# bg5sbk/dragonboat

Measured on AMD Instinct MI355X. Metric: quorum-commit decisions/sec (whole node) + % HBM roofline at 1/2/4/8 GPUs, higher is better.
Workload: dtype u64

## Files before the change

dragonboat_amd/csrc/hq_dstep_k.h:

```cpp
#pragma once

#include <chrono>
#include <cstdlib>

#include "hq_dstep.h"
#include "hq_internal.h"

namespace hq {
struct StepArgs {};
struct JobArgs {};
}

namespace {

enum List { kCommits, kReady, kResps, kStates, kDropped, kDeferred, kFallback, kDecisions,
            kRerun, kEvents, kSlotted, kLists };
enum InputError : uint32_t { kErrHandle = 1, kErrOffsets = 2, kErrBoffsets = 4, kErrTwice = 8,
                             kErrScan = 16, kErrTicket = 32 };
constexpr uint32_t kTickets = 8;

struct StepK : hq::StepArgs {
    hq_dgroup *groups;
    hq_dmember *members;
    hq_dread *reads;
    uint64_t n;
    uint64_t i_begin, i_end;
    uint64_t n_handles;
    uint64_t n_events, n_bytes;
    uint32_t *stamp;
    uint32_t step_no;
    uint32_t *error;
    uint32_t *wide;
    const uint32_t *handles;
    const uint64_t *offsets;
    const hq_event *events;
    const uint64_t *boffsets;
    const uint8_t *bytes;
    const uint64_t *prefix;
    uint64_t own_lo, own_hi;
    uint32_t *counts;
    uint32_t *wsum;
    uint64_t ws;
    const uint32_t *scan;
    uint64_t nw;
    uint32_t *pre;
    char *out;
    const struct Layout *layout;
    hq_dgroup *groups_old;
    uint64_t *match_old;
    hq_dread *reads_old;
    uint32_t spec_col, spec_valid;
    uint8_t *rerun;
    hq_ready_to_read *ready_slot;
    uint32_t *rerun_list;
    uint64_t out_cap;
    uint32_t allow_column, pad_j;
    struct Layout *host_layout;
    const uint32_t *sizes;
    const uint32_t *sizes_src;
    uint64_t *bsum;
    uint32_t spec_ready, chunk;
    uint64_t ready_off;
    uint32_t *ready_wide;
    uint64_t *tiles;
    uint32_t *tickets;
    const uint16_t *sizes16;
    const uint16_t *sizes16_src;
    uint32_t bytes_only;
    uint32_t slots;
    uint64_t slot_off, cnt_off;
    uint32_t test_scan_fail, pad_t;
};

constexpr uint32_t kSlotTile = 256;
constexpr uint64_t kSlotTileBytes = kSlotTile * sizeof(hq_ready_compact);
static_assert(kSlotTileBytes % 256 == 0, "slot tiles keep the region's 256-byte alignment");

struct Layout {
    uint64_t off[kLists];
    uint32_t len[kLists];
    uint64_t total;
    uint32_t error, overflow;
    uint32_t commit_column;
    uint32_t ready_compact;
    uint32_t pad;
    uint64_t reserve;
};
constexpr uint32_t kColumn64 = 1, kColumn32 = 2;
constexpr uint32_t kReadyCompact = 4;
constexpr uint32_t kReadySlots = 8;

constexpr uint32_t kTileVal = (1u << 28) - 1;

constexpr uint32_t kMaxJobs = kDStepMaxJobs;
struct JobMap : hq::JobArgs {
    const StepK *ks;
    uint32_t job0, count;
    uint32_t blk0[kMaxJobs + 1];
    uint32_t *tickets;
    uint32_t chunk;
    StepK *table_out;
    uint32_t bsum_scanned, pad;
};
static_assert(sizeof(StepK) % 8 == 0, "k_size_sums copies the table in 8-byte words");

__device__ __forceinline__ uint32_t job_of(const JobMap &m, uint32_t b) {
    uint32_t j = 0;
    while (j + 1 < m.count && b >= m.blk0[j + 1]) ++j;
    return j;
}

constexpr int kMaxChunks = 4;
constexpr int kMaxJobChunks = 8;
static_assert(kMaxChunks <= kMaxJobChunks, "the chunk events serve both paths");
static_assert(kMaxJobChunks <= kTickets, "a ticket word per pass A launch");
constexpr uint64_t kChunkGroups = 65536;
__host__ __device__ inline uint64_t slot_layout(uint64_t n, uint64_t *slot_off, uint64_t *cnt_off) {
    const uint64_t tiles = (n + kSlotTile - 1) / kSlotTile;
    const uint64_t so = (n * 4 + 255) & ~uint64_t(255);
    const uint64_t co = so + tiles * kSlotTileBytes;
    if (slot_off) *slot_off = so;
    if (cnt_off) *cnt_off = co;
    return co + ((tiles * 4 + 255) & ~uint64_t(255));
}

constexpr int kScanT = 1024, kScanE = 11;
constexpr uint64_t kScanSmall = 2 * kScanT * kScanE;

constexpr uint32_t kSizeTile = 1024;
constexpr uint64_t kSizeApplyDirect = 2048;

template <class K, class... A>
int launch(hq_ctx *ctx, hipStream_t s, const char *what, K k, uint64_t grid, unsigned block,
           const A &...a) {
    hipLaunchKernelGGL(k, dim3((unsigned)grid), dim3(block), 0, s, a...);
    return hq::check_hip(ctx, hipGetLastError(), what);
}

}

namespace hq {
int launch_step(hq_ctx *ctx, bool write, bool stream, bool small, const StepArgs &k);
int launch_step_jobs(hq_ctx *ctx, bool write, bool small, const JobArgs &m);
int launch_step_lite(hq_ctx *ctx, hipStream_t s, const StepArgs &k);
int launch_step_lite_jobs(hq_ctx *ctx, hipStream_t s, const JobArgs &m);
int launch_step_restore(hq_ctx *ctx, hipStream_t s, const StepArgs &k);
int launch_layout(hq_ctx *ctx, hipStream_t s, const StepArgs &k);
int launch_scan_layout(hq_ctx *ctx, hipStream_t s, const StepArgs &k);
int launch_scan_layout_jobs(hq_ctx *ctx, hipStream_t s, const JobArgs &m);
int launch_size_sums(hq_ctx *ctx, hipStream_t s, const JobArgs &m);
int launch_bsum_scan_jobs(hq_ctx *ctx, hipStream_t s, const JobArgs &m);
int launch_size_apply(hq_ctx *ctx, hipStream_t s, const JobArgs &m);
int scan_wave_sums(hq_ctx *ctx, hipStream_t s, void *tmp, size_t *tmp_bytes, uint32_t *wsum,
                   uint32_t *scan, size_t ws);
int scan_sizes(hq_ctx *ctx, hipStream_t s, void *tmp, size_t *tmp_bytes, const void *sizes,
               bool s16, uint64_t n, uint64_t *prefix);
inline uint64_t now_ns() {
    using namespace std::chrono;
    return (uint64_t)duration_cast<nanoseconds>(steady_clock::now().time_since_epoch()).count();
}
inline bool env_flag(const char *name) {
    const char *v = std::getenv(name);
    return v && std::atoi(v) != 0;
}
int grow(hq_ctx *ctx, void **p, size_t *cap, size_t need, bool keep, const char *what);
template <class T>
int grow(hq_ctx *ctx, T **p, size_t *cap, size_t need, bool keep, const char *what) {
    return grow(ctx, reinterpret_cast<void **>(p), cap, need, keep, what);
}
int stamp_clock(hq_dstep *d, hipStream_t s, int slot);
int wait_stream(hq_dstep *d, hipStream_t s, const char *what);
}

struct hq_dstep {
    hq_ctx *ctx = nullptr;
    bool test_fail_regrow = false;
    bool test_scan_fail = false;
    hq_dgroup *groups = nullptr;
    hq_dread *reads = nullptr;
    hq_dmember *members = nullptr;
    hq_dgroup *groups_old = nullptr;
    hq_dread *reads_old = nullptr;
    uint64_t *match_old = nullptr;
    uint8_t *rerun = nullptr;
    uint32_t *rerun_list = nullptr;
    hq_ready_to_read *ready_slot = nullptr;
    size_t rcap = 0;
    uint32_t *stamp = nullptr;
    uint64_t gcap = 0, mcap = 0;
    uint64_t n_groups = 0;
    uint32_t max_members = 0;
    uint32_t step_no = 0;
    uint32_t commit_column = 0;
    void *in = nullptr;
    size_t in_cap = 0;
    uint32_t *counts = nullptr, *scan = nullptr, *bases = nullptr;
    size_t cnt_cap = 0;
    uint32_t *wsum = nullptr;
    size_t wsum_cap = 0;
    bool wsum_dirty = true;
    void *scan_tmp = nullptr;
    size_t scan_tmp_cap = 0;
    void *host_out = nullptr;
    size_t host_out_cap = 0;
    Layout *layout = nullptr;
    Layout *host_layout = nullptr;
    hipStream_t copy = nullptr;
    hipEvent_t ev_in[kMaxJobChunks] = {};
    hipStream_t copy2 = nullptr;
    hipEvent_t ev_in2[kMaxJobChunks] = {};
    char *bounce = nullptr;
    hipEvent_t bounce_ev[2] = {nullptr, nullptr};
    hipEvent_t ev_sync = nullptr;
    hipEvent_t ev_t0 = nullptr, ev_t1 = nullptr;
    StepK *jobs_host = nullptr, *jobs_dev = nullptr;
    const StepK *jobs_host_dev = nullptr;
    uint32_t jobs_cap = 0;
    uint32_t *tickets = nullptr;
    bool tickets_dirty = false;
    uint64_t *tiles = nullptr;
    size_t tiles_cap = 0;
    uint32_t wait_mode = HQ_WAIT_BLOCK, wait_poll_us = 50, wait_sleep_us = 20;
    uint64_t wait_pred_ns = 0;
    bool wait_clock = false;
    uint64_t *clock_host = nullptr;
    hq_wait_clock last_wait{};
};
```

dragonboat_amd/csrc/hq_dstep_layout.hip:

```cpp
#include <hipcub/hipcub.hpp>

#include "hq_dstep_k.h"

namespace {

struct PackSize {
    const uint32_t *sizes;
    uint64_t n;
    const uint16_t *sizes16 = nullptr;
    __host__ __device__ uint64_t operator()(uint64_t i) const {
        if (sizes16) return i < n ? sizes16[i] : 0;
        const uint32_t s = i < n ? sizes[i] : 0;
        return (uint64_t)(s & 0xFFFFu) << 32 | (s >> 16);
    }
};

__device__ void layout_from(const uint32_t *bnd, uint64_t n, uint32_t *error, uint64_t cap,
                            uint32_t allow_column, uint64_t want_events, Layout *lay,
                            Layout *host_lay) {
    uint32_t *wide = error + 1;
    uint32_t *ready_wide = error + 2;
    if (want_events != ~uint64_t(0) && (uint64_t)(bnd[kEvents + 1] - bnd[kEvents]) != want_events)
        *error |= kErrBoffsets;
    lay->ready_compact = (allow_column & kReadyCompact) && !*ready_wide;
    const uint64_t rec[kLists] = {sizeof(hq_commit_event),
                                  lay->ready_compact ? sizeof(hq_ready_compact) : sizeof(hq_ready_to_read),
                                  sizeof(hq_read_index_resp), sizeof(hq_state_change),
                                  sizeof(hq_dropped_read), 8, 8, 0, 0, 0, 0};
    const uint32_t commits = bnd[1] - bnd[0];
    lay->commit_column = (allow_column & kColumn32) && !*wide && 4 * (uint64_t)commits > n
                             ? kColumn32
                         : (allow_column & kColumn64) && 2 * (uint64_t)commits > n ? kColumn64 : 0;
    const bool slots = (allow_column & kReadySlots) != 0;
    const uint64_t reserve = slots ? slot_layout(n, nullptr, nullptr) : 0;
    uint64_t total = reserve;
    for (int l = 0; l < kLists; ++l) {
        const uint32_t len = bnd[l + 1] - bnd[l];
        lay->len[l] = len;
        if (l == kCommits && slots && lay->commit_column == kColumn32) {
            lay->off[l] = 0;
            continue;
        }
        lay->off[l] = total;
        const uint64_t bytes = l == kCommits && lay->commit_column
                                   ? n * (lay->commit_column == kColumn32 ? 4 : 8)
                                   : len * rec[l];
        total += (bytes + 255) & ~uint64_t(255);
    }
    lay->total = total;
    lay->reserve = reserve;
    lay->error = *error;
    lay->overflow = total > cap;
    if (!((lay->overflow && !*error) || *error == kErrScan)) {
        *error = 0;
        *wide = 0;
        *ready_wide = 0;
    }
    *host_lay = *lay;
}

__global__ void k_layout(const uint32_t *scan, uint64_t n, uint64_t nw, uint32_t *error,
                         uint64_t cap, uint32_t allow_column, uint64_t want_events, Layout *lay,
                         Layout *host_lay) {
    if (threadIdx.x != 0) return;
    uint32_t bnd[kLists + 1];
    for (int l = 0; l <= kLists; ++l) bnd[l] = scan[(uint64_t)l * nw];
    layout_from(bnd, n, error, cap, allow_column, want_events, lay, host_lay);
}

__device__ __forceinline__ void scan_layout(const uint32_t *wsum, uint32_t *scan, uint64_t ws,
                                            uint64_t n, uint64_t nw, uint32_t *error, uint64_t cap,
                                            uint32_t allow_column, uint64_t want_events, Layout *lay,
                                            Layout *host_lay) {
    __shared__ uint32_t tile[kScanT * kScanE];
    __shared__ uint32_t wtot[kScanT / 64];
    __shared__ uint32_t bnd[kLists + 1];
    const int t = threadIdx.x, lane = t & 63, wv = t >> 6;
    uint32_t carry = 0;
    for (uint64_t base = 0; base < ws; base += (uint64_t)kScanT * kScanE) {
        for (int k = 0; k < kScanE; ++k) {
            const uint64_t j = base + (uint64_t)k * kScanT + t;
            tile[k * kScanT + t] = j < ws ? wsum[j] : 0u;
        }
        __syncthreads();
        uint32_t v[kScanE], sum = 0;
        for (int k = 0; k < kScanE; ++k) {
            v[k] = tile[t * kScanE + k];
            sum += v[k];
        }
        uint32_t x = sum;
        for (int d = 1; d < 64; d <<= 1) {
            const uint32_t y = __shfl_up(x, d, 64);
            x += lane >= d ? y : 0u;
        }
        if (lane == 63) wtot[wv] = x;
        __syncthreads();
        uint32_t before = 0, all = 0;
        for (int w = 0; w < kScanT / 64; ++w) {
            const uint32_t z = wtot[w];
            before += w < wv ? z : 0u;
            all += z;
        }
        uint32_t run = carry + before + x - sum;
        for (int k = 0; k < kScanE; ++k) {
            tile[t * kScanE + k] = run;
            run += v[k];
        }
        __syncthreads();
        for (int k = 0; k < kScanE; ++k) {
            const uint64_t j = base + (uint64_t)k * kScanT + t;
            if (j < ws) {
                const uint32_t e = tile[k * kScanT + t];
                scan[j] = e;
                if (j % nw == 0 && j / nw <= kLists) bnd[j / nw] = e;
            }
        }
        carry += all;
        __syncthreads();
    }
    if (t == 0) layout_from(bnd, n, error, cap, allow_column, want_events, lay, host_lay);
}

__global__ __launch_bounds__(kScanT) void k_scan_layout(const uint32_t *wsum, uint32_t *scan,
                                                        uint64_t ws, uint64_t n, uint64_t nw,
                                                        uint32_t *error, uint64_t cap,
                                                        uint32_t allow_column, uint64_t want_events,
                                                        Layout *lay, Layout *host_lay) {
    scan_layout(wsum, scan, ws, n, nw, error, cap, allow_column, want_events, lay, host_lay);
}

__host__ __device__ inline uint64_t want_events_of(const StepK &a) {
    return a.bytes_only ? a.n_events : ~uint64_t(0);
}

__global__ __launch_bounds__(kScanT) void k_scan_layout_jobs(const StepK *ks) {
    const StepK &a = ks[blockIdx.x];
    scan_layout(a.wsum, const_cast<uint32_t *>(a.scan), a.ws, a.n, a.nw, a.error, a.out_cap,
                a.allow_column, want_events_of(a), const_cast<Layout *>(a.layout), a.host_layout);
}

__device__ __forceinline__ uint64_t packed_size(const StepK &a, uint64_t i) {
    if (i >= a.n) return 0;
    if (a.bytes_only) return a.sizes16[i];
    const uint32_t s = a.sizes[i];
    return (uint64_t)(s & 0xFFFFu) << 32 | (s >> 16);
}

__device__ __forceinline__ uint64_t block_excl_scan(uint64_t v, uint64_t *total) {
    __shared__ uint64_t wt[1024 / 64];
    const int lane = threadIdx.x & 63, wv = threadIdx.x >> 6;
    uint64_t x = v;
#pragma unroll
    for (int d = 1; d < 64; d <<= 1) {
        const uint64_t y = __shfl_up(x, d, 64);
        x += lane >= d ? y : 0ull;
    }
    if (lane == 63) wt[wv] = x;
    __syncthreads();
    uint64_t before = 0, all = 0;
    for (int w = 0; w < (int)(blockDim.x / 64); ++w) {
        before += w < wv ? wt[w] : 0ull;
        all += wt[w];
    }
    __syncthreads();
    *total = all;
    return before + x - v;
}

__global__ __launch_bounds__(256) void k_size_sums(const JobMap m) {
    if (m.table_out && blockIdx.x == 0) {
        const uint64_t *src = reinterpret_cast<const uint64_t *>(m.ks + m.job0);
        uint64_t *dst = reinterpret_cast<uint64_t *>(m.table_out + m.job0);
        for (uint32_t q = threadIdx.x; q < m.count * (uint32_t)(sizeof(StepK) / 8); q += 256)
            dst[q] = src[q];
    }
    const uint32_t j = job_of(m, blockIdx.x);
    const StepK &a = m.ks[m.job0 + j];
    const uint64_t b = blockIdx.x - m.blk0[j], i0 = b * kSizeTile + threadIdx.x * 4;
    uint64_t v = 0;
    if (a.bytes_only && a.sizes16_src) {
        uint16_t *dst = const_cast<uint16_t *>(a.sizes16);
        uint16_t z[4];
        if (i0 + 4 <= a.n && !(reinterpret_cast<uintptr_t>(a.sizes16_src) & 7)) {
            const uint64_t w = *reinterpret_cast<const uint64_t *>(a.sizes16_src + i0);
#pragma unroll
            for (int k = 0; k < 4; ++k) z[k] = (uint16_t)(w >> (16 * k));
            *reinterpret_cast<uint64_t *>(dst + i0) = w;
        } else {
#pragma unroll
            for (int k = 0; k < 4; ++k) {
                const uint64_t i = i0 + k;
                z[k] = i < a.n ? a.sizes16_src[i] : 0;
                if (i < a.n) dst[i] = z[k];
            }
        }
#pragma unroll
        for (int k = 0; k < 4; ++k) v += z[k];
    } else if (!a.bytes_only && a.sizes_src) {
        uint32_t *dst = const_cast<uint32_t *>(a.sizes);
#pragma unroll
        for (int k = 0; k < 4; ++k) {
            const uint64_t i = i0 + k;
            const uint32_t z = i < a.n ? a.sizes_src[i] : 0;
            if (i < a.n) dst[i] = z;
            v += (uint64_t)(z & 0xFFFFu) << 32 | (z >> 16);
        }
    } else {
#pragma unroll
        for (int k = 0; k < 4; ++k) v += packed_size(a, i0 + k);
    }
    uint64_t tot;
    (void)block_excl_scan(v, &tot);
    if (threadIdx.x == 0) a.bsum[b] = tot;
}

__global__ __launch_bounds__(1024) void k_bsum_scan_jobs(const JobMap m) {
    const StepK &a = m.ks[m.job0 + blockIdx.x];
    const uint64_t nb = (a.n + 1 + kSizeTile - 1) / kSizeTile;
    uint64_t carry = 0;
    for (uint64_t base = 0; base < nb; base += 1024) {
        const uint64_t k = base + threadIdx.x;
        const uint64_t v = k < nb ? a.bsum[k] : 0;
        uint64_t tot;
        const uint64_t ex = block_excl_scan(v, &tot);
        if (k < nb) a.bsum[k] = carry + ex;
        carry += tot;
    }
}

__global__ __launch_bounds__(256) void k_size_apply(const JobMap m) {
    const uint32_t j = job_of(m, blockIdx.x);
    const StepK &a = m.ks[m.job0 + j];
    const uint64_t b = blockIdx.x - m.blk0[j], i0 = b * kSizeTile + threadIdx.x * 4;
    uint64_t base;
    if (m.bsum_scanned) {
        base = a.bsum[b];
    } else {
        uint64_t before = 0;
        for (uint64_t k = threadIdx.x; k < b; k += 256) before += a.bsum[k];
        (void)block_excl_scan(before, &base);
    }
    uint64_t v[4], sum = 0;
#pragma unroll
    for (int k = 0; k < 4; ++k) {
        v[k] = packed_size(a, i0 + k);
        sum += v[k];
    }
    uint64_t tot;
    uint64_t run = base + block_excl_scan(sum, &tot);
    uint64_t *prefix = const_cast<uint64_t *>(a.prefix);
#pragma unroll
    for (int k = 0; k < 4; ++k) {
        if (i0 + k <= a.n) prefix[i0 + k] = run;
        run += v[k];
    }
}

}

namespace hq {

int launch_layout(hq_ctx *ctx, hipStream_t s, const StepArgs &ka) {
    const StepK &k = static_cast<const StepK &>(ka);
    return launch(ctx, s, "k_layout", k_layout, 1, 64, k.scan, k.n, k.nw, k.error, k.out_cap,
                  k.allow_column, want_events_of(k), const_cast<Layout *>(k.layout), k.host_layout);
}
int launch_scan_layout(hq_ctx *ctx, hipStream_t s, const StepArgs &ka) {
    const StepK &k = static_cast<const StepK &>(ka);
    return launch(ctx, s, "k_scan_layout", k_scan_layout, 1, kScanT, k.wsum,
                  const_cast<uint32_t *>(k.scan), k.ws, k.n, k.nw, k.error, k.out_cap,
                  k.allow_column, want_events_of(k), const_cast<Layout *>(k.layout), k.host_layout);
}
int launch_scan_layout_jobs(hq_ctx *ctx, hipStream_t s, const JobArgs &ma) {
    const JobMap &m = static_cast<const JobMap &>(ma);
    return launch(ctx, s, "k_scan_layout_jobs", k_scan_layout_jobs, m.count, kScanT, m.ks);
}
int launch_size_sums(hq_ctx *ctx, hipStream_t s, const JobArgs &ma) {
    const JobMap &m = static_cast<const JobMap &>(ma);
    return launch(ctx, s, "k_size_sums", k_size_sums, m.blk0[m.count], 256, m);
}
int launch_bsum_scan_jobs(hq_ctx *ctx, hipStream_t s, const JobArgs &ma) {
    const JobMap &m = static_cast<const JobMap &>(ma);
    return launch(ctx, s, "k_bsum_scan_jobs", k_bsum_scan_jobs, m.count, 1024, m);
}
int launch_size_apply(hq_ctx *ctx, hipStream_t s, const JobArgs &ma) {
    const JobMap &m = static_cast<const JobMap &>(ma);
    return launch(ctx, s, "k_size_apply", k_size_apply, m.blk0[m.count], 256, m);
}

int scan_wave_sums(hq_ctx *ctx, hipStream_t s, void *tmp, size_t *tmp_bytes, uint32_t *wsum,
                   uint32_t *scan, size_t ws) {
    return check_hip(ctx, hipcub::DeviceScan::ExclusiveSum(tmp, *tmp_bytes, wsum, scan, ws, s),
                     tmp ? "hipcub scan" : "hipcub scan size");
}
int scan_sizes(hq_ctx *ctx, hipStream_t s, void *tmp, size_t *tmp_bytes, const void *sizes,
               bool s16, uint64_t n, uint64_t *prefix) {
    const hipcub::TransformInputIterator<uint64_t, PackSize, hipcub::CountingInputIterator<uint64_t>>
        packed_sizes(hipcub::CountingInputIterator<uint64_t>(0),
                     PackSize{static_cast<const uint32_t *>(sizes), n,
                              s16 ? static_cast<const uint16_t *>(sizes) : nullptr});
    return check_hip(ctx, hipcub::DeviceScan::ExclusiveSum(tmp, *tmp_bytes, packed_sizes, prefix,
                                                           n + 1, s),
                     tmp ? "hipcub scan" : "hipcub scan size");
}

}
```

dragonboat_amd/csrc/hq_dstep_step.hip:

```cpp
#include "hq_dstep_k.h"
#include "hq_launch.h"

namespace {

__device__ __forceinline__ bool is_response(uint32_t t) {
    return t == HQ_MSG_REPLICATE_RESP || t == HQ_MSG_REQUEST_VOTE_RESP ||
           t == HQ_MSG_HEARTBEAT_RESP || t == 20 || t == 8 || t == 9;
}

struct ByteReader {
    const uint8_t *p, *end;
    uintptr_t wa = 1;
    uint64_t w = 0;

    __device__ __forceinline__ bool more() const { return p < end; }
    __device__ __forceinline__ uint32_t next() {
        const uintptr_t a = reinterpret_cast<uintptr_t>(p);
        if ((a & ~uintptr_t(7)) != wa) {
            wa = a & ~uintptr_t(7);
            w = *reinterpret_cast<const uint64_t *>(wa);
        }
        ++p;
        return (uint32_t)(w >> (8 * (a & 7))) & 0xFF;
    }
};

__device__ __forceinline__ bool dvar(ByteReader &r, uint64_t &v) {
    v = 0;
    for (int sh = 0; sh < 64; sh += 7) {
        if (!r.more()) return false;
        const uint32_t b = r.next();
        v |= (uint64_t)(b & 0x7F) << sh;
        if (b < 0x80) return true;
    }
    return false;
}

struct DPrev {
    uint64_t term = 0, index = 0, hint = 0, high = 0;
    bool have_index = false;
    uint32_t last = 0, run = 0, run_from = 0;
};

__device__ bool decode_event(ByteReader &r, DPrev &pv, hq_event &v) {
    v = hq_event{};
    if (pv.run == 0) {
        if (!r.more()) return false;
        const uintptr_t a = reinterpret_cast<uintptr_t>(r.p);
        if ((a & ~uintptr_t(7)) != r.wa) {
            r.wa = a & ~uintptr_t(7);
            r.w = *reinterpret_cast<const uint64_t *>(r.wa);
        }
        const uint32_t h0 = (uint32_t)(r.w >> (8 * (a & 7))) & 0xFF;
        if ((h0 & 7) == HQ_EV_MESSAGE && ((h0 >> 3) & 7) == 6) {
            (void)r.next();
            uint64_t m;
            if (!(pv.last & 3) || !dvar(r, m) || m == 0 || m > 0xFFFF) return false;
            pv.run = (uint32_t)m;
            pv.last &= 7u;
            if (h0 & 0x80) {
                uint64_t f0;
                if (!dvar(r, f0) || f0 > 0xFFFFFFFFull - m) return false;
                pv.run_from = (uint32_t)f0;
                pv.last |= 8u;
            }
        }
    }
    if (pv.run) {
        --pv.run;
        v.kind = HQ_EV_MESSAGE;
        v.type = (pv.last & 3) == 1 ? HQ_MSG_REPLICATE_RESP : HQ_MSG_HEARTBEAT_RESP;
        v.reject = (pv.last >> 2) & 1;
        v.term = pv.term;
        if ((pv.last & 3) == 1) {
            v.log_index = pv.index;
        } else {
            v.hint = pv.hint;
            v.hint_high = pv.high;
        }
        if (pv.last & 8u) {
            v.from = pv.run_from++;
            return true;
        }
        return dvar(r, v.from);
    }
    const uint32_t h = r.next();
    v.kind = h & 7;
    if (v.kind == HQ_EV_READ) return dvar(r, v.hint) && dvar(r, v.hint_high);
    if (v.kind == HQ_EV_PROPOSE) return dvar(r, v.log_index);
    if (v.kind != HQ_EV_MESSAGE) return true;
    const uint32_t code = (h >> 3) & 7;
    uint64_t t = code == 0 || code == 4 ? HQ_MSG_REPLICATE_RESP
               : code == 1 ? HQ_MSG_REQUEST_VOTE_RESP
               : code == 2 || code == 5 ? HQ_MSG_HEARTBEAT_RESP
               : code == 3 ? HQ_MSG_READ_INDEX : 0;
    if (code == 7 && !dvar(r, t)) return false;
    if (code == 4 && !pv.have_index) return false;
    v.type = (uint32_t)t;
    v.reject = (h >> 6) & 1;
    if (!dvar(r, v.from)) return false;
    if (!(h & 0x80) && !dvar(r, pv.term)) return false;
    v.term = pv.term;
    if ((code == 0 || code == 7) && !dvar(r, v.log_index)) return false;
    if (code == 4) v.log_index = pv.index;
    if ((code == 2 || code == 3 || code == 7) && !(dvar(r, v.hint) && dvar(r, v.hint_high)))
        return false;
    if (code == 5) {
        v.hint = pv.hint;
        v.hint_high = pv.high;
    }
    if (code == 0 || code == 4) {
        pv.index = v.log_index;
        pv.have_index = true;
    }
    if (code == 2 || code == 5) {
        pv.hint = v.hint;
        pv.high = v.hint_high;
    }
    pv.last = (code == 0 || code == 4 ? 1u : code == 2 || code == 5 ? 2u : 0u) | v.reject << 2;
    return true;
}

constexpr uint32_t kStageReady = 64;
constexpr uint32_t kStageBytes = 16384;

constexpr uint64_t kScanWaitTicks = 10000000;
__device__ __forceinline__ uint64_t tile_word(uint32_t step, uint32_t chunk, bool incl, uint32_t v) {
    return (uint64_t)step << 32 | (uint64_t)(chunk & 7) << 29 | (uint64_t)incl << 28 | (v & kTileVal);
}
__device__ __forceinline__ uint64_t tile_load(const uint64_t *p) {
    return __hip_atomic_load(p, __ATOMIC_RELAXED, __HIP_MEMORY_SCOPE_AGENT);
}
__device__ __forceinline__ void tile_store(uint64_t *p, uint64_t v) {
    __hip_atomic_store(p, v, __ATOMIC_RELAXED, __HIP_MEMORY_SCOPE_AGENT);
}

__device__ __forceinline__ uint32_t draw_ticket(uint32_t *ctr) {
    __shared__ uint32_t t;
    if (threadIdx.x == 0) t = atomicAdd(ctr, 1u);
    __syncthreads();
    return t;
}

template <bool WRITE, int MC>
struct Engine {
    const StepK &a;
    uint64_t i;
    hq_dgroup g;
    const hq_dmember *gm;
    uint64_t match[MC];
    uint64_t ids[MC];
    uint32_t active;
    hq_dread *rd;
    uint32_t cnt[kLists];
    uint32_t base[kLists];
    hq_ready_to_read *stage = nullptr;
    uint32_t stage_lo = 0;
    uint64_t c0 = 0;
    bool slotted = false;

    __device__ __forceinline__ Engine(const StepK &k, uint64_t idx, uint32_t h, hq_dread *reads)
        : a(k), i(idx), rd(reads) {
        g = WRITE ? k.groups_old[h] : k.groups[h];
        gm = k.members + g.mem;
        active = 0;
#pragma unroll
        for (uint32_t s = 0; s < MC; ++s) {
            match[s] = 0;
            ids[s] = 0;
            if (s < g.n_members) {
                match[s] = WRITE ? k.match_old[g.mem + s] : gm[s].match;
                ids[s] = gm[s].node_id;
                active |= (uint32_t)(WRITE ? (g.pad1 >> s) & 1 : gm[s].active != 0) << s;
            }
        }
        const hq_dread *rs = (WRITE ? k.reads_old : k.reads) + (uint64_t)h * kDReads;
        for (uint32_t r = 0; r < g.n_reads; ++r) rd[r] = rs[r];
        for (int l = 0; l < kLists; ++l) {
            cnt[l] = 0;
            base[l] = WRITE ? k.scan[(uint64_t)l * k.nw + (idx >> 6)] - k.scan[(uint64_t)l * k.nw] +
                                  k.pre[(uint64_t)l * k.n + idx]
                            : 0;
        }
    }

    __device__ __forceinline__ uint32_t quorum() const { return g.n_voting / 2 + 1; }
    __device__ __forceinline__ int member_of(uint64_t id) const {
        int m = -1;
#pragma unroll
        for (int s = MC - 1; s >= 0; --s)
            m = (s < (int)g.n_members && ids[s] == id) ? s : m;
        return m;
    }
    __device__ __forceinline__ uint64_t match_of(int mi) const {
        uint64_t v = 0;
#pragma unroll
        for (int s = 0; s < (int)MC; ++s) v = s == mi ? match[s] : v;
        return v;
    }
    __device__ __forceinline__ void set_match(int mi, uint64_t v) {
#pragma unroll
        for (int s = 0; s < (int)MC; ++s) match[s] = s == mi ? v : match[s];
    }
    __device__ __forceinline__ uint32_t slot(int l) { return base[l] + cnt[l]++; }
    template <class T>
    __device__ __forceinline__ T *list(int l) const {
        return reinterpret_cast<T *>(a.out + a.layout->off[l]);
    }

    __device__ __forceinline__ void ready(uint64_t index, uint64_t low, uint64_t high) {
        if (WRITE && slotted) return;
        const uint32_t p = slot(kReady);
        const hq_ready_to_read r{g.cluster_id, index, low, high};
        const int64_t delta = (int64_t)(index - c0);
        if (!WRITE) {
            if (p == 0) a.ready_slot[i] = r;
            if (a.ready_wide && delta != (int64_t)(int32_t)delta) atomicOr(a.ready_wide, 1u);
        } else if (a.layout->ready_compact) {
            list<hq_ready_compact>(kReady)[p] =
                hq_ready_compact{low, high, (uint32_t)i, (int32_t)delta};
        } else if (stage && p - stage_lo < kStageReady) {
            stage[p - stage_lo] = r;
        } else {
            list<hq_ready_to_read>(kReady)[p] = r;
        }
    }
    __device__ __forceinline__ void resp(uint64_t to, uint64_t index, uint64_t hint, uint64_t high) {
        const uint32_t p = slot(kResps);
        if (WRITE)
            list<hq_read_index_resp>(kResps)[p] = hq_read_index_resp{g.cluster_id, to, index, hint, high};
    }
    __device__ __forceinline__ void state_change(uint32_t reason) {
        const uint32_t p = slot(kStates);
        if (WRITE) list<hq_state_change>(kStates)[p] = hq_state_change{g.cluster_id, g.term, g.state, reason};
    }
    __device__ __forceinline__ void dropped(uint64_t low, uint64_t high, uint64_t from, uint32_t reason) {
        const uint32_t p = slot(kDropped);
        if (WRITE)
            list<hq_dropped_read>(kDropped)[p] = hq_dropped_read{g.cluster_id, low, high, from, reason, 0};
    }
    __device__ __forceinline__ void defer(uint64_t e) {
        const uint32_t p = slot(kDeferred);
        if (WRITE) list<uint64_t>(kDeferred)[p] = e;
    }

    __device__ __forceinline__ void reset(uint64_t term) {
        g.term = term;
        g.granted = g.rejected = 0;
        g.n_reads = 0;
#pragma unroll
        for (uint32_t s = 0; s < MC; ++s)
            match[s] = s < g.n_members && ids[s] == g.node_id ? g.last : 0;
        active = 0;
    }
    __device__ __forceinline__ void become_follower(uint64_t term, uint32_t reason) {
        g.state = HQ_STATE_FOLLOWER;
        reset(term);
        state_change(reason);
    }
    __device__ __forceinline__ void become_leader() {
        g.state = HQ_STATE_LEADER;
        reset(g.term);
        state_change(HQ_REASON_VOTE);
        g.term_start = g.last + 1;
        g.last += 1;
        match[0] = g.last;
        if (g.n_voting == 1) try_commit();
    }

    __device__ __forceinline__ void try_commit() {
        static_assert(HQ_MAX_VOTERS == 8, "the network sorts 8 voting slots");
        cnt[kDecisions]++;
        const uint32_t n = g.n_voting, q = quorum();
        uint64_t v[8];
#pragma unroll
        for (uint32_t s = 0; s < 8; ++s) v[s] = s < n ? match[s] : 0;
        auto cx = [&](int i, int j) {
            const uint64_t a = v[i], b = v[j];
            const bool gt = a > b;
            v[i] = gt ? a : b;
            v[j] = gt ? b : a;
        };
        cx(0, 2); cx(1, 3); cx(4, 6); cx(5, 7);
        cx(0, 4); cx(1, 5); cx(2, 6); cx(3, 7);
        cx(0, 1); cx(2, 3); cx(4, 5); cx(6, 7);
        cx(2, 4); cx(3, 5);
        cx(1, 4); cx(3, 6);
        cx(1, 2); cx(3, 4); cx(5, 6);
        uint64_t best = 0;
#pragma unroll
        for (uint32_t s = 0; s < 8; ++s) best = s + 1 == q ? v[s] : best;
        if (best > g.committed && best >= g.term_start && best <= g.last)
            g.committed = best;
    }

    __device__ __forceinline__ bool read_index(uint64_t from, uint64_t low, uint64_t high, uint64_t e) {
        if (g.state != HQ_STATE_LEADER) {
            defer(e);
            return true;
        }
        const int fm = member_of(from);
        const uint32_t role = fm >= 0 ? gm[fm].role : 0xFF;
        if (role == HQ_ROLE_WITNESS) {
            dropped(low, high, from, HQ_DROP_WITNESS);
            return true;
        }
        if (g.n_voting == 1) {
            ready(g.committed, low, high);
            if (from != g.node_id && role == HQ_ROLE_OBSERVER) resp(from, g.committed, low, high);
            return true;
        }
        if (!(g.committed >= g.term_start && g.committed <= g.last)) {
            dropped(low, high, from, HQ_DROP_NOT_READY);
            return true;
        }
        for (uint32_t k = 0; k < g.n_reads; ++k)
            if (rd[k].low == low && rd[k].high == high) return true;
        if (g.n_reads && g.committed < rd[g.n_reads - 1].index) return false;
        if (g.n_reads >= kDReads) return false;
        hq_dread &r = rd[g.n_reads++];
        r = hq_dread{};
        r.index = g.committed;
        r.from = from;
        r.low = low;
        r.high = high;
        return true;
    }

    __device__ __forceinline__ bool confirm(uint64_t hint, uint64_t high, int mi) {
        uint32_t k = 0;
        while (k < g.n_reads && !(rd[k].low == hint && rd[k].high == high)) ++k;
        if (k == g.n_reads) return true;
        if (mi >= (int)g.n_voting) return false;
        rd[k].confirmed |= (uint8_t)(1u << mi);
        cnt[kDecisions]++;
        if ((uint32_t)__popc(rd[k].confirmed) + 1 < quorum()) return true;
        const uint64_t index = rd[k].index;
        for (uint32_t r = 0; r <= k; ++r) {
            if (rd[r].from == 0 || rd[r].from == g.node_id) ready(index, rd[r].low, rd[r].high);
            else resp(rd[r].from, index, hint, high);
        }
        for (uint32_t r = k + 1; r < g.n_reads; ++r) rd[r - k - 1] = rd[r];
        g.n_reads -= (uint8_t)(k + 1);
        return true;
    }

    __device__ __forceinline__ bool handle(const hq_event &ev, uint64_t e) {
        switch (ev.kind) {
        case HQ_EV_READ:
            return read_index(0, ev.hint, ev.hint_high, e);
        case HQ_EV_CHECK_QUORUM: {
            if (g.state != HQ_STATE_LEADER) return true;
            cnt[kDecisions]++;
            const uint32_t vm = (1u << g.n_voting) - 1u;
            const bool has = (uint32_t)__popc((active | 1u) & vm) >= quorum();
            active &= ~vm;
            if (!has) become_follower(g.term, HQ_REASON_CHECK_QUORUM);
            return true;
        }
        case HQ_EV_ELECTION:
            if (g.state == HQ_STATE_LEADER) return true;
            g.state = HQ_STATE_CANDIDATE;
            reset(g.term + 1);
            state_change(HQ_REASON_CAMPAIGN);
            g.granted = 1;
            cnt[kDecisions]++;
            if (g.n_voting == 1) become_leader();
            return true;
        case HQ_EV_PROPOSE:
            if (g.state != HQ_STATE_LEADER) {
                defer(e);
                return true;
            }
            g.last += ev.log_index;
            if (match[0] < g.last) match[0] = g.last;
            if (g.n_voting == 1) try_commit();
            return true;
        case HQ_EV_MESSAGE:
            break;
        default:
            return false;
        }
        const uint32_t type = ev.type;
        if (type != HQ_MSG_REPLICATE_RESP && type != HQ_MSG_HEARTBEAT_RESP &&
            type != HQ_MSG_REQUEST_VOTE_RESP && type != HQ_MSG_READ_INDEX)
            return false;
        const int mi = member_of(ev.from);
        if (mi < 0 && is_response(type)) return true;
        if (ev.term != 0 && ev.term != g.term) {
            if (ev.term < g.term) return true;
            become_follower(ev.term, HQ_REASON_HIGHER_TERM);
        }
        if (g.state == HQ_STATE_LEADER) {
            switch (type) {
            case HQ_MSG_REPLICATE_RESP:
                if (!ev.reject && match_of(mi) < ev.log_index) {
                    if (ev.log_index > g.last) return false;
                    set_match(mi, ev.log_index);
                    try_commit();
                }
                active |= 1u << mi;
                return true;
            case HQ_MSG_HEARTBEAT_RESP:
                if (ev.hint != 0 && !confirm(ev.hint, ev.hint_high, mi)) return false;
                active |= 1u << mi;
                return true;
            case HQ_MSG_READ_INDEX:
                return read_index(ev.from, ev.hint, ev.hint_high, e);
            default:
                return true;
            }
        }
        if (g.state == HQ_STATE_CANDIDATE && type == HQ_MSG_REQUEST_VOTE_RESP) {
            if (mi >= (int)g.n_voting) return true;
            const uint8_t bit = (uint8_t)(1u << mi);
            if (!((g.granted | g.rejected) & bit)) {
                if (ev.reject) g.rejected |= bit;
                else g.granted |= bit;
            }
            cnt[kDecisions]++;
            const uint32_t q = quorum();
            if ((uint32_t)__popc(g.granted) == q) become_leader();
            else if ((uint32_t)__popc(g.rejected) == q)
                become_follower(g.term, HQ_REASON_VOTE);
            return true;
        }
        if (type == HQ_MSG_READ_INDEX) return read_index(ev.from, ev.hint, ev.hint_high, e);
        return true;
    }

    template <bool STREAM>
    __device__ __forceinline__ void run(uint64_t e0, uint64_t e1, const uint8_t *p, const uint8_t *end) {
        const uint64_t committed0 = c0 = g.committed;
        DPrev pv;
        ByteReader br{p, end};
        const bool by_bytes = STREAM && a.bytes_only;
        uint64_t e = e0;
        for (;; ++e) {
            if (by_bytes ? !(br.more() || pv.run) : e >= e1) break;
            hq_event ev;
            bool dec = true;
            if (STREAM && (by_bytes || !(g.flags & kDSuspended))) dec = decode_event(br, pv, ev);
            if (by_bytes && !dec) {
                if (!WRITE) atomicOr(a.error, (uint32_t)kErrBoffsets);
                break;
            }
            if (g.flags & kDSuspended) {
                defer(e);
                continue;
            }
            bool ok;
            if (STREAM) {
                ok = dec && handle(ev, e);
            } else {
                ev = a.events[e];
                ok = handle(ev, e);
            }
            if (!ok) {
                g.flags |= kDSuspended;
                const uint32_t p = slot(kFallback);
                if (WRITE) list<uint64_t>(kFallback)[p] = g.cluster_id;
                defer(e);
            } else if (STREAM && pv.run) {
                e += take_run(pv, by_bytes ? ~0ull : e1 - e - 1);
            }
        }
        cnt[kEvents] = (uint32_t)(e - e0);
        if (STREAM && !WRITE && !by_bytes && !(g.flags & kDSuspended) && (br.p != br.end || pv.run))
            atomicOr(a.error, (uint32_t)kErrBoffsets);
        if (!WRITE && g.committed - committed0 > 0xFFFFFFFFull && a.wide)
            atomicOr(a.wide, 1u);
        if (!WRITE && a.spec_col)
            reinterpret_cast<uint32_t *>(a.out)[i] = (uint32_t)(g.committed - committed0);
        if (WRITE && a.layout->commit_column) {
        } else if (g.committed != committed0) {
            const uint32_t p = slot(kCommits);
            if (WRITE) list<hq_commit_event>(kCommits)[p] = hq_commit_event{g.cluster_id, g.committed};
        }
    }

    __device__ __forceinline__ uint32_t take_run(DPrev &pv, uint64_t room) {
        const uint32_t kind = pv.last & 3;
        const bool rej = (pv.last >> 2) & 1;
        if (!(pv.last & 8u) || pv.run > room || g.state != HQ_STATE_LEADER || (g.flags & kDSuspended) ||
            (pv.term != 0 && pv.term != g.term) ||
            !(kind == 2 ? pv.hint == 0 : (rej || pv.index <= g.last)))
            return 0;
        const uint32_t m = pv.run;
        uint32_t upd = 0;
        for (uint32_t j = 0; j < m; ++j) {
            const int mi = member_of(pv.run_from + j);
            if (mi < 0) continue;
            if (kind == 1 && !rej && match_of(mi) < pv.index) {
                set_match(mi, pv.index);
                ++upd;
            }
            active |= 1u << mi;
        }
        pv.run_from += m;
        pv.run = 0;
        if (upd) {
            try_commit();
            cnt[kDecisions] += upd - 1;
        }
        return m;
    }

    __device__ __forceinline__ void save_old(uint32_t h) {
        hq_dgroup o = g;
        o.pad1 = active;
        a.groups_old[h] = o;
#pragma unroll
        for (uint32_t s = 0; s < MC; ++s)
            if (s < g.n_members) a.match_old[g.mem + s] = match[s];
        for (uint32_t r = 0; r < g.n_reads; ++r) a.reads_old[(uint64_t)h * kDReads + r] = rd[r];
    }

    __device__ __forceinline__ void store(uint32_t h) {
        a.groups[h] = g;
        hq_dmember *m = a.members + g.mem;
#pragma unroll
        for (uint32_t s = 0; s < MC; ++s) {
            if (s < g.n_members) {
                m[s].match = match[s];
                m[s].active = (uint8_t)((active >> s) & 1);
            }
        }
        for (uint32_t r = 0; r < g.n_reads; ++r) a.reads[(uint64_t)h * kDReads + r] = rd[r];
    }
};

__device__ void ready_tail(const StepK &a, uint64_t tile, uint32_t chunk, bool member, bool first,
                          uint64_t i, uint32_t cnt, bool one, uint4 *sbuf) {
    __shared__ uint32_t s_w[256 / 64], s_excl, s_any, s_first, s_ok;
    __shared__ unsigned long long s_first_i;
    const int lane = threadIdx.x & 63, wv = threadIdx.x >> 6;
    if (threadIdx.x == 0) {
        s_any = 0;
        s_first = 0;
    }
    uint32_t x = cnt;
#pragma unroll
    for (int d = 1; d < 64; d <<= 1) {
        const uint32_t y = __shfl_up(x, d, 64);
        x += lane >= d ? y : 0u;
    }
    if (lane == 63) s_w[wv] = x;
    __syncthreads();
    if (member) s_any = 1;
    if (first) {
        s_first = 1;
        s_first_i = i;
    }
    uint32_t before = 0, agg = 0;
#pragma unroll
    for (int w = 0; w < 256 / 64; ++w) {
        before += w < wv ? s_w[w] : 0u;
        agg += s_w[w];
    }
    __syncthreads();
    if (!s_any) return;
    if (wv == 0) {
        const uint32_t step = a.step_no;
        uint32_t excl = 0;
        bool ok = true;
        if (s_first) {
            if (s_first_i > 0) {
                const uint64_t w = tile_load(a.tiles + (s_first_i - 1) / 256);
                ok = (uint32_t)(w >> 32) == step && ((w >> 28) & 1) &&
                     (uint32_t)((w >> 29) & 7) < chunk;
                excl = (uint32_t)w & kTileVal;
            }
        } else if (tile == 0 || a.test_scan_fail) {
            ok = false;
        } else {
            if (lane == 0) tile_store(a.tiles + tile, tile_word(step, chunk, false, agg));
            int64_t hi = (int64_t)tile - 1;
            const uint64_t t_wait = wall_clock64();
            for (;;) {
                const int64_t p = hi - lane;
                const uint64_t w = p >= 0 ? tile_load(a.tiles + p) : 0;
                const bool ready = p >= 0 && (uint32_t)(w >> 32) == step &&
                                   (uint32_t)((w >> 29) & 7) == (chunk & 7);
                const uint64_t rdy = __ballot(ready), inc = __ballot(ready && ((w >> 28) & 1));
                const uint64_t need = inc ? (inc & (0 - inc)) * 2 - 1 : ~0ull;
                if ((rdy & need) == need) {
                    uint32_t v = (lane < 64 - __clzll((long long)need) || !inc) && ready
                                     ? (uint32_t)w & kTileVal : 0u;
#pragma unroll
                    for (int d = 32; d >= 1; d >>= 1) v += __shfl_xor(v, d, 64);
                    excl += v;
                    if (inc) break;
                    hi -= 64;
                    if (hi < 0) {
                        ok = false;
                        break;
                    }
                    continue;
                }
                if (wall_clock64() - t_wait > kScanWaitTicks) {
                    ok = false;
                    break;
                }
                __builtin_amdgcn_s_sleep(1);
            }
        }
        if (lane == 0) {
            if (!ok) atomicOr(a.error, (uint32_t)kErrScan);
            tile_store(a.tiles + tile, tile_word(step, chunk, true, excl + agg));
            s_excl = excl;
            s_ok = ok;
        }
    }
    __syncthreads();
    const uint32_t lo = s_excl;
    if (!s_ok || agg == 0 || a.ready_off + (uint64_t)(lo + agg) * sizeof(hq_ready_to_read) > a.out_cap)
        return;
    constexpr uint32_t kCap = kStageBytes / sizeof(hq_ready_to_read);
    hq_ready_to_read *stage = reinterpret_cast<hq_ready_to_read *>(sbuf);
    hq_ready_to_read *dst = reinterpret_cast<hq_ready_to_read *>(a.out + a.ready_off) + lo;
    const uint32_t pos = before + x - cnt;
    if (one) {
        const hq_ready_to_read r = a.ready_slot[i];
        if (pos < kCap) stage[pos] = r;
        else dst[pos] = r;
    }
    __syncthreads();
    const uint32_t nq = 2 * min(agg, kCap);
    const uint4 *src = reinterpret_cast<const uint4 *>(stage);
    uint4 *out = reinterpret_cast<uint4 *>(dst);
    for (uint32_t q = threadIdx.x; q < nq; q += 256) out[q] = src[q];
}

__device__ void slot_store(const StepK &a, uint64_t tile, bool slotted, const hq_ready_compact &rec,
                           uint4 *buf) {
    __shared__ uint32_t s_w[256 / 64];
    const int lane = threadIdx.x & 63, wv = threadIdx.x >> 6;
    const uint64_t bal = __ballot(slotted);
    if (lane == 0) s_w[wv] = (uint32_t)__popcll(bal);
    __syncthreads();
    uint32_t before = 0, agg = 0;
#pragma unroll
    for (int w = 0; w < 256 / 64; ++w) {
        before += w < wv ? s_w[w] : 0u;
        agg += s_w[w];
    }
    hq_ready_compact *stage = reinterpret_cast<hq_ready_compact *>(buf);
    if (slotted) stage[before + __popcll(bal & ((1ull << lane) - 1))] = rec;
    __syncthreads();
    char *dst = a.out + a.slot_off + tile * kSlotTileBytes;
    const uint32_t nbytes = agg * (uint32_t)sizeof(hq_ready_compact);
    for (uint32_t q = threadIdx.x; q < nbytes / 16; q += 256)
        reinterpret_cast<uint4 *>(dst)[q] = buf[q];
    if (threadIdx.x == 0) {
        if (nbytes & 8)
            reinterpret_cast<uint2 *>(dst)[nbytes / 8 - 1] =
                reinterpret_cast<const uint2 *>(buf)[nbytes / 8 - 1];
        reinterpret_cast<uint32_t *>(a.out + a.cnt_off)[tile] = agg;
    }
}

template <bool WRITE, bool STREAM, int MC>
__device__ __forceinline__ void step_groups(const StepK &a, uint64_t blk, uint32_t chunk = 0) {
    __shared__ uint32_t wtot[WRITE ? 1 : 256 / 64][kLists];
    if (!WRITE && (threadIdx.x & 63) < kLists) wtot[threadIdx.x >> 6][threadIdx.x & 63] = 0;
    uint64_t i = a.i_begin + blk * 256 + threadIdx.x;
    constexpr bool STAGE = !WRITE && STREAM;
    bool act = true;
    if (WRITE && (a.layout->error | a.layout->overflow)) return;
    if (WRITE && a.layout->commit_column) {
        if (i >= a.layout->len[kRerun]) return;
        i = a.rerun_list[i];
    } else if (i >= a.i_end) {
        if (!STAGE) return;
        act = false;
    }
    uint64_t e0 = 0, e1 = 0, b0 = 0, b1 = 0;
    if (act && STREAM && a.prefix) {
        const uint64_t x0 = a.prefix[i], x1 = a.prefix[i + 1];
        e0 = x0 >> 32;
        e1 = x1 >> 32;
        b0 = x0 & 0xFFFFFFFFu;
        b1 = x1 & 0xFFFFFFFFu;
        if (!WRITE) {
            if (i + 1 == a.n && a.own_lo == 0 &&
                ((!a.bytes_only && e1 != a.n_events) || b1 != a.n_bytes))
                atomicOr(a.error, (uint32_t)kErrBoffsets);
            if (b1 < a.own_lo || b1 >= a.own_hi) act = false;
        }
    } else if (act) {
        e0 = a.offsets[i];
        e1 = a.offsets[i + 1];
        if (STREAM) {
            b0 = a.boffsets[i];
            b1 = a.boffsets[i + 1];
        }
    }
    if (!STAGE && !act) return;
    const bool member = act;
    const bool first = member && (a.prefix ? i == 0 || b0 < a.own_lo : i == a.i_begin);
    const uint32_t h = !act ? 0u : a.handles ? a.handles[i] : (uint32_t)i;
    if (!WRITE && act) {
        uint32_t err = 0;
        if (h >= a.n_handles) err |= kErrHandle;
        if (e1 < e0 || (!STREAM && e1 > a.n_events) || (STREAM && a.prefix && e1 > a.n_events))
            err |= kErrOffsets;
        if (STREAM && (b1 < b0 || b1 > a.n_bytes)) err |= kErrBoffsets;
        if (!(err & kErrHandle) && atomicExch(a.stamp + h, a.step_no) == a.step_no)
            err |= kErrTwice;
        if (err) {
            atomicOr(a.error, err);
            for (int l = 0; l < kLists; ++l) a.counts[(uint64_t)l * a.n + i] = 0;
            a.rerun[i] = 0;
            act = false;
        }
    }
    const uint8_t *src0 = a.bytes + b0;
    __shared__ uint4 sbuf[STAGE ? kStageBytes / 16 : 1];
    if constexpr (STAGE) {
        __shared__ unsigned long long s_lo, s_hi;
        if (threadIdx.x == 0) {
            s_lo = ~0ull;
            s_hi = 0;
        }
        __syncthreads();
        const uint64_t base = reinterpret_cast<uint64_t>(a.bytes);
        if (act && b1 > b0) {
            atomicMin(&s_lo, (unsigned long long)(base + b0));
            atomicMax(&s_hi, (unsigned long long)(base + b1));
        }
        __syncthreads();
        const uint64_t lo = s_lo & ~15ull, hi = (s_hi + 15) & ~15ull;
        const bool fits = s_hi > s_lo && hi - lo <= kStageBytes;
        if (fits) {
            constexpr int kU = kStageBytes / (256 * 16);
            uint4 v[kU];
#pragma unroll
            for (int u = 0; u < kU; ++u) {
                const uint64_t o = (threadIdx.x + 256ull * u) * 16;
                if (o < hi - lo) v[u] = *reinterpret_cast<const uint4 *>(lo + o);
            }
#pragma unroll
            for (int u = 0; u < kU; ++u) {
                const uint64_t o = (threadIdx.x + 256ull * u) * 16;
                if (o < hi - lo) sbuf[o / 16] = v[u];
            }
        }
        __syncthreads();
        if (act && fits) src0 = reinterpret_cast<const uint8_t *>(sbuf) + (base + b0 - lo);
    }
    uint32_t n_ready = 0;
    bool one_ready = false, slotted = false;
    hq_ready_compact srec{};
    if (act) {
        hq_dread reads[kDReads];
        Engine<WRITE, MC> eng(a, i, h, reads);
        if (!WRITE) eng.save_old(h);
        if (WRITE && STREAM && a.bytes_only) e0 = eng.base[kEvents];
        if (WRITE && a.slots) eng.slotted = (a.rerun[i] & 8) != 0;
        __shared__ hq_ready_to_read stage[WRITE ? 256 / 64 : 1][WRITE ? kStageReady : 1];
        const bool staged = WRITE && !a.layout->commit_column && !a.layout->ready_compact;
        if (staged) {
            eng.stage = stage[threadIdx.x >> 6];
            eng.stage_lo = __builtin_amdgcn_readfirstlane(eng.base[kReady]);
        }
        if (STREAM)
            eng.template run<true>(e0, e1, src0, src0 + (b1 - b0));
        else
            eng.template run<false>(e0, e1, nullptr, nullptr);
        if (staged) {
            const uint64_t act = __ballot(1);
            const int last = 63 - __clzll((long long)act);
            const uint32_t end = __shfl(eng.base[kReady] + eng.cnt[kReady], last);
            const uint32_t nrec = min(end - eng.stage_lo, kStageReady);
            const uint32_t rank = __popcll(act & ((1ull << (threadIdx.x & 63)) - 1));
            const uint32_t nact = __popcll(act);
            asm volatile("s_waitcnt lgkmcnt(0)" ::: "memory");
            __builtin_amdgcn_wave_barrier();
            const uint4 *src = reinterpret_cast<const uint4 *>(eng.stage);
            uint4 *dst = reinterpret_cast<uint4 *>(eng.template list<hq_ready_to_read>(kReady) +
                                                   eng.stage_lo);
            for (uint32_t q = rank; q < 2 * nrec; q += nact) dst[q] = src[q];
        }
        if (!WRITE) {
            const bool others = (eng.cnt[kResps] | eng.cnt[kStates] | eng.cnt[kDropped] |
                                 eng.cnt[kDeferred] | eng.cnt[kFallback]) != 0;
            const bool rerun = others || eng.cnt[kReady] > 1;
            one_ready = !rerun && eng.cnt[kReady] == 1;
            if (a.slots && one_ready) {
                const hq_ready_to_read r = a.ready_slot[i];
                const int64_t delta = (int64_t)(r.index - eng.c0);
                if (delta == (int64_t)(int32_t)delta) {
                    slotted = true;
                    one_ready = false;
                    srec = hq_ready_compact{r.ctx_low, r.ctx_high, (uint32_t)i, (int32_t)delta};
                    eng.cnt[kReady] = 0;
                    eng.cnt[kSlotted] = 1;
                }
            }
            n_ready = eng.cnt[kReady];
            eng.cnt[kRerun] = rerun;
            for (int l = 0; l < kLists; ++l) a.counts[(uint64_t)l * a.n + i] = eng.cnt[l];
            a.rerun[i] = (uint8_t)(2 | rerun | (one_ready ? 4 : 0) | (slotted ? 8 : 0));
            eng.store(h);
            uint32_t *wt = wtot[threadIdx.x >> 6];
            for (int l = 0; l < kLists; ++l)
                if (eng.cnt[l]) atomicAdd(wt + l, eng.cnt[l]);
            asm volatile("s_waitcnt lgkmcnt(0)" ::: "memory");
            __builtin_amdgcn_wave_barrier();
            if ((int)(threadIdx.x & 63) == __ffsll((long long)__ballot(1)) - 1) {
                for (int l = 0; l < kLists; ++l) {
                    const uint32_t v = wt[l];
                    if (v) atomicAdd(a.wsum + (uint64_t)l * a.nw + (i >> 6), v);
                }
            }
        }
    }
    if constexpr (STAGE) {
        if (a.spec_ready)
            ready_tail(a, (a.i_begin >> 8) + blk, chunk, member, first, i, n_ready, one_ready, sbuf);
        else if (a.slots)
            slot_store(a, (a.i_begin >> 8) + blk, slotted, srec, sbuf);
    }
}

template <bool WRITE, bool STREAM, int MC>
__global__ __launch_bounds__(256) void k_step(const StepK a) {
    if constexpr (!WRITE && STREAM) {
        const uint32_t b = draw_ticket(a.tickets + a.chunk);
        if (b >= gridDim.x) {
            if (threadIdx.x == 0) atomicOr(a.error, (uint32_t)kErrTicket);
            return;
        }
        step_groups<WRITE, STREAM, MC>(a, b, a.chunk);
    } else {
        step_groups<WRITE, STREAM, MC>(a, blockIdx.x);
    }
}

template <bool WRITE, bool STREAM, int MC>
__global__ __launch_bounds__(256) void k_step_jobs(const JobMap m) {
    uint32_t b = blockIdx.x;
    if constexpr (!WRITE && STREAM) {
        b = draw_ticket(m.tickets + m.chunk);
        if (b >= gridDim.x) {
            if (threadIdx.x == 0) atomicOr(m.ks[m.job0].error, (uint32_t)kErrTicket);
            return;
        }
    }
    const uint32_t j = job_of(m, b);
    step_groups<WRITE, STREAM, MC>(m.ks[m.job0 + j], b - m.blk0[j], m.chunk);
}

__device__ __forceinline__ void lite_groups(const StepK &a, uint64_t blk, uint32_t *tickets) {
    const uint64_t i = blk * 256 + threadIdx.x;
    if (tickets && threadIdx.x < kTickets) tickets[threadIdx.x] = 0;
    if (i < a.ws) a.wsum[i] = 0;
    __shared__ __align__(16) hq_ready_to_read stage[256 / 64][kStageReady];
    static_assert(sizeof(stage) >= kSlotTileBytes, "the slot staging fits the list's");
    if (a.slots && !a.spec_valid && !(a.layout->error | a.layout->overflow)) {
        const bool s = i < a.n && (a.rerun[i] & 8);
        hq_ready_compact rec{};
        if (s) {
            const hq_ready_to_read r = a.ready_slot[i];
            const uint32_t h = a.handles ? a.handles[i] : (uint32_t)i;
            rec = hq_ready_compact{r.ctx_low, r.ctx_high, (uint32_t)i,
                                   (int32_t)(int64_t)(r.index - a.groups_old[h].committed)};
        }
        slot_store(a, blk, s, rec, reinterpret_cast<uint4 *>(&stage[0][0]));
        __syncthreads();
    }
    const bool in = i < a.n;
    if ((a.layout->error | a.layout->overflow) || !__ballot(in)) return;
    const uint32_t col = a.layout->commit_column;
    const uint8_t rr = in ? a.rerun[i] : 0;
    const int lane = threadIdx.x & 63;
    const bool replay = in && (!col || (rr & 1));
    const bool any = __ballot(replay) != 0;
    uint32_t pre_ready = 0, pre_rerun = 0;
    for (int l = 0; l < kLists; ++l) {
        if (!any && l != kReady && l != kRerun) continue;
        const uint32_t c = in ? a.counts[(uint64_t)l * a.n + i] : 0;
        uint32_t x = c;
#pragma unroll
        for (int d = 1; d < 64; d <<= 1) {
            const uint32_t y = __shfl_up(x, d, 64);
            x += lane >= d ? y : 0u;
        }
        if (replay) a.pre[(uint64_t)l * a.n + i] = x - c;
        if (l == kReady) pre_ready = x - c;
        if (l == kRerun) pre_rerun = x - c;
    }
    if (!col) return;
    const bool col32 = col == kColumn32;
    if (!(col32 && a.spec_valid && a.spec_ready)) {
        constexpr uint64_t l = kReady;
        const uint64_t w = i >> 6;
        const uint32_t lo = a.scan[l * a.nw + w] - a.scan[l * a.nw];
        const uint32_t cnt = a.scan[l * a.nw + w + 1] - a.scan[l * a.nw + w];
        hq_ready_to_read *st = stage[threadIdx.x >> 6];
        const uint32_t pos = lo + pre_ready;
        const uint32_t nrec = min(cnt, kStageReady);
        if (a.layout->ready_compact) {
            hq_ready_compact *stc = reinterpret_cast<hq_ready_compact *>(st);
            hq_ready_compact *dst = reinterpret_cast<hq_ready_compact *>(a.out + a.layout->off[kReady]);
            if (rr & 4) {
                const hq_ready_to_read r = a.ready_slot[i];
                const uint32_t h = a.handles ? a.handles[i] : (uint32_t)i;
                const hq_ready_compact c{r.ctx_low, r.ctx_high, (uint32_t)i,
                                         (int32_t)(int64_t)(r.index - a.groups_old[h].committed)};
                if (pos - lo < kStageReady) stc[pos - lo] = c;
                else dst[pos] = c;
            }
            asm volatile("s_waitcnt lgkmcnt(0)" ::: "memory");
            __builtin_amdgcn_wave_barrier();
            const uint2 *src = reinterpret_cast<const uint2 *>(stc);
            uint2 *out = reinterpret_cast<uint2 *>(dst + lo);
            for (uint32_t q = lane; q < 3 * nrec; q += 64) out[q] = src[q];
        } else {
            hq_ready_to_read *dst = reinterpret_cast<hq_ready_to_read *>(a.out + a.layout->off[kReady]);
            if (rr & 4) {
                if (pos - lo < kStageReady) st[pos - lo] = a.ready_slot[i];
                else dst[pos] = a.ready_slot[i];
            }
            asm volatile("s_waitcnt lgkmcnt(0)" ::: "memory");
            __builtin_amdgcn_wave_barrier();
            const uint4 *src = reinterpret_cast<const uint4 *>(st);
            uint4 *out = reinterpret_cast<uint4 *>(dst + lo);
            for (uint32_t q = lane; q < 2 * nrec; q += 64) out[q] = src[q];
        }
    }
    if (!in) return;
    if (!(col32 && a.spec_valid)) {
        const uint32_t h = a.handles ? a.handles[i] : (uint32_t)i;
        const uint64_t c0 = a.groups_old[h].committed, c1 = a.groups[h].committed;
        char *cw = a.out + a.layout->off[kCommits];
        if (col32)
            reinterpret_cast<uint32_t *>(cw)[i] = (uint32_t)(c1 - c0);
        else
            reinterpret_cast<uint64_t *>(cw)[i] = c1 != c0 ? c1 : 0;
    }
    if (rr & 1) {
        const uint64_t l = kRerun;
        a.rerun_list[a.scan[l * a.nw + (i >> 6)] - a.scan[l * a.nw] + pre_rerun] = (uint32_t)i;
    }
}

__global__ __launch_bounds__(256) void k_step_lite(const StepK a) {
    lite_groups(a, blockIdx.x, blockIdx.x == 0 ? a.tickets : nullptr);
}

__global__ __launch_bounds__(256) void k_step_lite_jobs(const JobMap m) {
    const uint32_t j = job_of(m, blockIdx.x);
    lite_groups(m.ks[m.job0 + j], blockIdx.x - m.blk0[j], blockIdx.x == 0 ? m.tickets : nullptr);
}

__global__ __launch_bounds__(256) void k_step_restore(const StepK a) {
    const uint64_t i = (uint64_t)blockIdx.x * 256 + threadIdx.x;
    if (i >= a.n || !(a.rerun[i] & 2)) return;
    const uint32_t h = a.handles ? a.handles[i] : (uint32_t)i;
    hq_dgroup g = a.groups_old[h];
    const uint32_t act = g.pad1;
    g.pad1 = 0;
    a.groups[h] = g;
    for (uint32_t s = 0; s < g.n_members; ++s) {
        a.members[g.mem + s].match = a.match_old[g.mem + s];
        a.members[g.mem + s].active = (uint8_t)((act >> s) & 1);
    }
    for (uint32_t r = 0; r < g.n_reads; ++r)
        a.reads[(uint64_t)h * kDReads + r] = a.reads_old[(uint64_t)h * kDReads + r];
}

}

namespace hq {

int launch_step(hq_ctx *ctx, bool write, bool stream, bool small, const StepArgs &ka) {
    const StepK &k = static_cast<const StepK &>(ka);
    const dim3 grid((unsigned)((k.i_end - k.i_begin + 255) / 256)), blk(256);
    int rc = pre_launch(ctx);
    if (rc) return rc;
    dispatch_bool(write, [&](auto w) {
        dispatch_bool(stream, [&](auto st) {
            dispatch<8, kDMembers>(small ? 8u : kDMembers, [&](auto mc) {
                hipLaunchKernelGGL((k_step<decltype(w)::value, decltype(st)::value,
                                           (int)decltype(mc)::value>),
                                   grid, blk, 0, ctx->stream, k);
            });
        });
    });
    return post_launch(ctx, write ? "k_step<write>" : "k_step<count>");
}

int launch_step_jobs(hq_ctx *ctx, bool write, bool small, const JobArgs &ma) {
    const JobMap &m = static_cast<const JobMap &>(ma);
    int rc = pre_launch(ctx);
    if (rc) return rc;
    dispatch_bool(write, [&](auto w) {
        dispatch<8, kDMembers>(small ? 8u : kDMembers, [&](auto mc) {
            hipLaunchKernelGGL((k_step_jobs<decltype(w)::value, true, (int)decltype(mc)::value>),
                               dim3(m.blk0[m.count]), dim3(256), 0, ctx->stream, m);
        });
    });
    return post_launch(ctx, write ? "k_step_jobs<write>" : "k_step_jobs<count>");
}

int launch_step_lite(hq_ctx *ctx, hipStream_t s, const StepArgs &ka) {
    const StepK &k = static_cast<const StepK &>(ka);
    return launch(ctx, s, "k_step_lite", k_step_lite, (k.n + 255) / 256, 256, k);
}
int launch_step_lite_jobs(hq_ctx *ctx, hipStream_t s, const JobArgs &ma) {
    const JobMap &m = static_cast<const JobMap &>(ma);
    return launch(ctx, s, "k_step_lite_jobs", k_step_lite_jobs, m.blk0[m.count], 256, m);
}
int launch_step_restore(hq_ctx *ctx, hipStream_t s, const StepArgs &ka) {
    const StepK &k = static_cast<const StepK &>(ka);
    return launch(ctx, s, "k_step_restore", k_step_restore, (k.n + 255) / 256, 256, k);
}

}
```

Before: 110.7 billion.

## Use explicit global address space loads/stores and scalar constant loads for job tables

```diff
diff --git a/dragonboat_amd/csrc/hq_dstep_k.h b/dragonboat_amd/csrc/hq_dstep_k.h
--- a/dragonboat_amd/csrc/hq_dstep_k.h
+++ b/dragonboat_amd/csrc/hq_dstep_k.h
@@ -2,6 +2,7 @@
 
 #include <chrono>
 #include <cstdlib>
+#include <type_traits>
 
 #include "hq_dstep.h"
 #include "hq_internal.h"
@@ -108,6 +109,67 @@
     uint32_t j = 0;
     while (j + 1 < m.count && b >= m.blk0[j + 1]) ++j;
     return j;
+}
+
+__device__ __forceinline__ StepK load_job(const StepK *p) {
+    static_assert(std::is_trivially_copyable<StepK>::value, "copied word by word");
+    const auto *src = (const __attribute__((address_space(4))) uint64_t *)p;
+    uint64_t w[sizeof(StepK) / 8];
+#pragma unroll
+    for (uint32_t k = 0; k < sizeof(StepK) / 8; ++k) w[k] = src[k];
+    StepK a;
+    __builtin_memcpy(&a, w, sizeof a);
+    return a;
+}
+
+#define HQ_GLOBAL __attribute__((address_space(1)))
+template <class T>
+struct GWord {
+    using type = std::conditional_t<
+        alignof(T) % 16 == 0 && sizeof(T) % 16 == 0, uint32_t __attribute__((ext_vector_type(4))),
+        std::conditional_t<alignof(T) % 8 == 0 && sizeof(T) % 8 == 0, uint64_t, uint32_t>>;
+};
+template <class T>
+__device__ __forceinline__ T gload(const T *p) {
+    if constexpr (std::is_arithmetic<T>::value) {
+        return *(const HQ_GLOBAL T *)p;
+    } else {
+        static_assert(std::is_trivially_copyable<T>::value && sizeof(T) % 4 == 0, "whole words");
+        using W = typename GWord<T>::type;
+        const auto *src = (const HQ_GLOBAL W *)p;
+        W w[sizeof(T) / sizeof(W)];
+#pragma unroll
+        for (uint32_t k = 0; k < sizeof(T) / sizeof(W); ++k) w[k] = src[k];
+        T v;
+        __builtin_memcpy(&v, w, sizeof v);
+        return v;
+    }
+}
+template <class T>
+__device__ __forceinline__ void gstore(T *p, const std::common_type_t<T> &v) {
+    if constexpr (std::is_arithmetic<T>::value) {
+        *(HQ_GLOBAL T *)p = v;
+    } else {
+        static_assert(std::is_trivially_copyable<T>::value && sizeof(T) % 4 == 0, "whole words");
+        using W = typename GWord<T>::type;
+        auto *dst = (HQ_GLOBAL W *)p;
+        W w[sizeof(T) / sizeof(W)];
+        __builtin_memcpy(w, &v, sizeof v);
+#pragma unroll
+        for (uint32_t k = 0; k < sizeof(T) / sizeof(W); ++k) dst[k] = w[k];
+    }
+}
+__device__ __forceinline__ uint32_t gexch(uint32_t *p, uint32_t v) {
+    return __hip_atomic_exchange((HQ_GLOBAL uint32_t *)p, v, __ATOMIC_RELAXED,
+                                 __HIP_MEMORY_SCOPE_AGENT);
+}
+__device__ __forceinline__ void gor(uint32_t *p, uint32_t v) {
+    (void)__hip_atomic_fetch_or((HQ_GLOBAL uint32_t *)p, v, __ATOMIC_RELAXED,
+                                __HIP_MEMORY_SCOPE_AGENT);
+}
+__device__ __forceinline__ uint32_t gadd(uint32_t *p, uint32_t v) {
+    return __hip_atomic_fetch_add((HQ_GLOBAL uint32_t *)p, v, __ATOMIC_RELAXED,
+                                  __HIP_MEMORY_SCOPE_AGENT);
 }
 
 constexpr int kMaxChunks = 4;
diff --git a/dragonboat_amd/csrc/hq_dstep_layout.hip b/dragonboat_amd/csrc/hq_dstep_layout.hip
--- a/dragonboat_amd/csrc/hq_dstep_layout.hip
+++ b/dragonboat_amd/csrc/hq_dstep_layout.hip
@@ -16,19 +16,23 @@
 };
 
 __device__ void layout_from(const uint32_t *bnd, uint64_t n, uint32_t *error, uint64_t cap,
-                            uint32_t allow_column, uint64_t want_events, Layout *lay,
+                            uint32_t allow_column, uint64_t want_events, Layout *dev_lay,
                             Layout *host_lay) {
     uint32_t *wide = error + 1;
     uint32_t *ready_wide = error + 2;
+    uint32_t err = gload(error);
+    const uint32_t is_wide = gload(wide), is_ready_wide = gload(ready_wide);
+    Layout l_{};
+    Layout *const lay = &l_;
     if (want_events != ~uint64_t(0) && (uint64_t)(bnd[kEvents + 1] - bnd[kEvents]) != want_events)
-        *error |= kErrBoffsets;
-    lay->ready_compact = (allow_column & kReadyCompact) && !*ready_wide;
+        err |= kErrBoffsets;
+    lay->ready_compact = (allow_column & kReadyCompact) && !is_ready_wide;
     const uint64_t rec[kLists] = {sizeof(hq_commit_event),
                                   lay->ready_compact ? sizeof(hq_ready_compact) : sizeof(hq_ready_to_read),
                                   sizeof(hq_read_index_resp), sizeof(hq_state_change),
                                   sizeof(hq_dropped_read), 8, 8, 0, 0, 0, 0};
     const uint32_t commits = bnd[1] - bnd[0];
-    lay->commit_column = (allow_column & kColumn32) && !*wide && 4 * (uint64_t)commits > n
+    lay->commit_column = (allow_column & kColumn32) && !is_wide && 4 * (uint64_t)commits > n
                              ? kColumn32
                          : (allow_column & kColumn64) && 2 * (uint64_t)commits > n ? kColumn64 : 0;
     const bool slots = (allow_column & kReadySlots) != 0;
@@ -49,14 +53,16 @@
     }
     lay->total = total;
     lay->reserve = reserve;
-    lay->error = *error;
+    lay->error = err;
     lay->overflow = total > cap;
-    if (!((lay->overflow && !*error) || *error == kErrScan)) {
-        *error = 0;
-        *wide = 0;
-        *ready_wide = 0;
-    }
-    *host_lay = *lay;
+    if (!((lay->overflow && !err) || err == kErrScan)) {
+        err = 0;
+        gstore(wide, 0u);
+        gstore(ready_wide, 0u);
+    }
+    gstore(error, err);
+    gstore(dev_lay, *lay);
+    gstore(host_lay, *lay);
 }
 
 __global__ void k_layout(const uint32_t *scan, uint64_t n, uint64_t nw, uint32_t *error,
@@ -64,7 +70,7 @@
                          Layout *host_lay) {
     if (threadIdx.x != 0) return;
     uint32_t bnd[kLists + 1];
-    for (int l = 0; l <= kLists; ++l) bnd[l] = scan[(uint64_t)l * nw];
+    for (int l = 0; l <= kLists; ++l) bnd[l] = gload(scan + (uint64_t)l * nw);
     layout_from(bnd, n, error, cap, allow_column, want_events, lay, host_lay);
 }
 
@@ -80,7 +86,7 @@
     for (uint64_t base = 0; base < ws; base += (uint64_t)kScanT * kScanE) {
         for (int k = 0; k < kScanE; ++k) {
             const uint64_t j = base + (uint64_t)k * kScanT + t;
-            tile[k * kScanT + t] = j < ws ? wsum[j] : 0u;
+            tile[k * kScanT + t] = j < ws ? gload(wsum + j) : 0u;
         }
         __syncthreads();
         uint32_t v[kScanE], sum = 0;
@@ -111,7 +117,7 @@
             const uint64_t j = base + (uint64_t)k * kScanT + t;
             if (j < ws) {
                 const uint32_t e = tile[k * kScanT + t];
-                scan[j] = e;
+                gstore(scan + j, e);
                 if (j % nw == 0 && j / nw <= kLists) bnd[j / nw] = e;
             }
         }
@@ -134,15 +140,15 @@
 }
 
 __global__ __launch_bounds__(kScanT) void k_scan_layout_jobs(const StepK *ks) {
-    const StepK &a = ks[blockIdx.x];
+    const StepK a = load_job(ks + blockIdx.x);
     scan_layout(a.wsum, const_cast<uint32_t *>(a.scan), a.ws, a.n, a.nw, a.error, a.out_cap,
                 a.allow_column, want_events_of(a), const_cast<Layout *>(a.layout), a.host_layout);
 }
 
 __device__ __forceinline__ uint64_t packed_size(const StepK &a, uint64_t i) {
     if (i >= a.n) return 0;
-    if (a.bytes_only) return a.sizes16[i];
-    const uint32_t s = a.sizes[i];
+    if (a.bytes_only) return gload(a.sizes16 + i);
+    const uint32_t s = gload(a.sizes + i);
     return (uint64_t)(s & 0xFFFFu) << 32 | (s >> 16);
 }
 
@@ -172,26 +178,26 @@
         const uint64_t *src = reinterpret_cast<const uint64_t *>(m.ks + m.job0);
         uint64_t *dst = reinterpret_cast<uint64_t *>(m.table_out + m.job0);
         for (uint32_t q = threadIdx.x; q < m.count * (uint32_t)(sizeof(StepK) / 8); q += 256)
-            dst[q] = src[q];
+            gstore(dst + q, gload(src + q));
     }
     const uint32_t j = job_of(m, blockIdx.x);
-    const StepK &a = m.ks[m.job0 + j];
+    const StepK a = load_job(m.ks + m.job0 + j);
     const uint64_t b = blockIdx.x - m.blk0[j], i0 = b * kSizeTile + threadIdx.x * 4;
     uint64_t v = 0;
     if (a.bytes_only && a.sizes16_src) {
         uint16_t *dst = const_cast<uint16_t *>(a.sizes16);
         uint16_t z[4];
         if (i0 + 4 <= a.n && !(reinterpret_cast<uintptr_t>(a.sizes16_src) & 7)) {
-            const uint64_t w = *reinterpret_cast<const uint64_t *>(a.sizes16_src + i0);
+            const uint64_t w = gload(reinterpret_cast<const uint64_t *>(a.sizes16_src + i0));
 #pragma unroll
             for (int k = 0; k < 4; ++k) z[k] = (uint16_t)(w >> (16 * k));
-            *reinterpret_cast<uint64_t *>(dst + i0) = w;
+            gstore(reinterpret_cast<uint64_t *>(dst + i0), w);
         } else {
 #pragma unroll
             for (int k = 0; k < 4; ++k) {
                 const uint64_t i = i0 + k;
-                z[k] = i < a.n ? a.sizes16_src[i] : 0;
-                if (i < a.n) dst[i] = z[k];
+                z[k] = i < a.n ? gload(a.sizes16_src + i) : 0;
+                if (i < a.n) gstore(dst + i, z[k]);
             }
         }
 #pragma unroll
@@ -201,8 +207,8 @@
 #pragma unroll
         for (int k = 0; k < 4; ++k) {
             const uint64_t i = i0 + k;
-            const uint32_t z = i < a.n ? a.sizes_src[i] : 0;
-            if (i < a.n) dst[i] = z;
+            const uint32_t z = i < a.n ? gload(a.sizes_src + i) : 0;
+            if (i < a.n) gstore(dst + i, z);
             v += (uint64_t)(z & 0xFFFFu) << 32 | (z >> 16);
         }
     } else {
@@ -211,33 +217,33 @@
     }
     uint64_t tot;
     (void)block_excl_scan(v, &tot);
-    if (threadIdx.x == 0) a.bsum[b] = tot;
+    if (threadIdx.x == 0) gstore(a.bsum + b, tot);
 }
 
 __global__ __launch_bounds__(1024) void k_bsum_scan_jobs(const JobMap m) {
-    const StepK &a = m.ks[m.job0 + blockIdx.x];
+    const StepK a = load_job(m.ks + m.job0 + blockIdx.x);
     const uint64_t nb = (a.n + 1 + kSizeTile - 1) / kSizeTile;
     uint64_t carry = 0;
     for (uint64_t base = 0; base < nb; base += 1024) {
         const uint64_t k = base + threadIdx.x;
-        const uint64_t v = k < nb ? a.bsum[k] : 0;
+        const uint64_t v = k < nb ? gload(a.bsum + k) : 0;
         uint64_t tot;
         const uint64_t ex = block_excl_scan(v, &tot);
-        if (k < nb) a.bsum[k] = carry + ex;
+        if (k < nb) gstore(a.bsum + k, carry + ex);
         carry += tot;
     }
 }
 
 __global__ __launch_bounds__(256) void k_size_apply(const JobMap m) {
     const uint32_t j = job_of(m, blockIdx.x);
-    const StepK &a = m.ks[m.job0 + j];
+    const StepK a = load_job(m.ks + m.job0 + j);
     const uint64_t b = blockIdx.x - m.blk0[j], i0 = b * kSizeTile + threadIdx.x * 4;
     uint64_t base;
     if (m.bsum_scanned) {
-        base = a.bsum[b];
+        base = gload(a.bsum + b);
     } else {
         uint64_t before = 0;
-        for (uint64_t k = threadIdx.x; k < b; k += 256) before += a.bsum[k];
+        for (uint64_t k = threadIdx.x; k < b; k += 256) before += gload(a.bsum + k);
         (void)block_excl_scan(before, &base);
     }
     uint64_t v[4], sum = 0;
@@ -251,7 +257,7 @@
     uint64_t *prefix = const_cast<uint64_t *>(a.prefix);
 #pragma unroll
     for (int k = 0; k < 4; ++k) {
-        if (i0 + k <= a.n) prefix[i0 + k] = run;
+        if (i0 + k <= a.n) gstore(prefix + (i0 + k), run);
         run += v[k];
     }
 }
diff --git a/dragonboat_amd/csrc/hq_dstep_step.hip b/dragonboat_amd/csrc/hq_dstep_step.hip
--- a/dragonboat_amd/csrc/hq_dstep_step.hip
+++ b/dragonboat_amd/csrc/hq_dstep_step.hip
@@ -129,15 +129,16 @@
     return (uint64_t)step << 32 | (uint64_t)(chunk & 7) << 29 | (uint64_t)incl << 28 | (v & kTileVal);
 }
 __device__ __forceinline__ uint64_t tile_load(const uint64_t *p) {
-    return __hip_atomic_load(p, __ATOMIC_RELAXED, __HIP_MEMORY_SCOPE_AGENT);
+    return __hip_atomic_load((const HQ_GLOBAL uint64_t *)p, __ATOMIC_RELAXED,
+                             __HIP_MEMORY_SCOPE_AGENT);
 }
 __device__ __forceinline__ void tile_store(uint64_t *p, uint64_t v) {
-    __hip_atomic_store(p, v, __ATOMIC_RELAXED, __HIP_MEMORY_SCOPE_AGENT);
+    __hip_atomic_store((HQ_GLOBAL uint64_t *)p, v, __ATOMIC_RELAXED, __HIP_MEMORY_SCOPE_AGENT);
 }
 
 __device__ __forceinline__ uint32_t draw_ticket(uint32_t *ctr) {
     __shared__ uint32_t t;
-    if (threadIdx.x == 0) t = atomicAdd(ctr, 1u);
+    if (threadIdx.x == 0) t = gadd(ctr, 1u);
     __syncthreads();
     return t;
 }
@@ -161,7 +162,7 @@
 
     __device__ __forceinline__ Engine(const StepK &k, uint64_t idx, uint32_t h, hq_dread *reads)
         : a(k), i(idx), rd(reads) {
-        g = WRITE ? k.groups_old[h] : k.groups[h];
+        g = gload(WRITE ? k.groups_old + h : k.groups + h);
         gm = k.members + g.mem;
         active = 0;
 #pragma unroll
@@ -169,17 +170,18 @@
             match[s] = 0;
             ids[s] = 0;
             if (s < g.n_members) {
-                match[s] = WRITE ? k.match_old[g.mem + s] : gm[s].match;
-                ids[s] = gm[s].node_id;
-                active |= (uint32_t)(WRITE ? (g.pad1 >> s) & 1 : gm[s].active != 0) << s;
+                match[s] = WRITE ? gload(k.match_old + g.mem + s) : gload(&gm[s].match);
+                ids[s] = gload(&gm[s].node_id);
+                active |= (uint32_t)(WRITE ? (g.pad1 >> s) & 1 : gload(&gm[s].active) != 0) << s;
             }
         }
         const hq_dread *rs = (WRITE ? k.reads_old : k.reads) + (uint64_t)h * kDReads;
-        for (uint32_t r = 0; r < g.n_reads; ++r) rd[r] = rs[r];
+        for (uint32_t r = 0; r < g.n_reads; ++r) rd[r] = gload(rs + r);
         for (int l = 0; l < kLists; ++l) {
             cnt[l] = 0;
-            base[l] = WRITE ? k.scan[(uint64_t)l * k.nw + (idx >> 6)] - k.scan[(uint64_t)l * k.nw] +
-                                  k.pre[(uint64_t)l * k.n + idx]
+            base[l] = WRITE ? gload(k.scan + (uint64_t)l * k.nw + (idx >> 6)) -
+                                  gload(k.scan + (uint64_t)l * k.nw) +
+                                  gload(k.pre + (uint64_t)l * k.n + idx)
                             : 0;
         }
     }
@@ -205,7 +207,7 @@
     __device__ __forceinline__ uint32_t slot(int l) { return base[l] + cnt[l]++; }
     template <class T>
     __device__ __forceinline__ T *list(int l) const {
-        return reinterpret_cast<T *>(a.out + a.layout->off[l]);
+        return reinterpret_cast<T *>(a.out + gload(&a.layout->off[l]));
     }
 
     __device__ __forceinline__ void ready(uint64_t index, uint64_t low, uint64_t high) {
@@ -214,34 +216,38 @@
         const hq_ready_to_read r{g.cluster_id, index, low, high};
         const int64_t delta = (int64_t)(index - c0);
         if (!WRITE) {
-            if (p == 0) a.ready_slot[i] = r;
-            if (a.ready_wide && delta != (int64_t)(int32_t)delta) atomicOr(a.ready_wide, 1u);
-        } else if (a.layout->ready_compact) {
-            list<hq_ready_compact>(kReady)[p] =
-                hq_ready_compact{low, high, (uint32_t)i, (int32_t)delta};
+            if (p == 0) gstore(a.ready_slot + i, r);
+            if (a.ready_wide && delta != (int64_t)(int32_t)delta) gor(a.ready_wide, 1u);
+        } else if (gload(&a.layout->ready_compact)) {
+            gstore(list<hq_ready_compact>(kReady) + p,
+                   hq_ready_compact{low, high, (uint32_t)i, (int32_t)delta});
         } else if (stage && p - stage_lo < kStageReady) {
             stage[p - stage_lo] = r;
         } else {
-            list<hq_ready_to_read>(kReady)[p] = r;
+            gstore(list<hq_ready_to_read>(kReady) + p, r);
         }
     }
     __device__ __forceinline__ void resp(uint64_t to, uint64_t index, uint64_t hint, uint64_t high) {
         const uint32_t p = slot(kResps);
         if (WRITE)
-            list<hq_read_index_resp>(kResps)[p] = hq_read_index_resp{g.cluster_id, to, index, hint, high};
+            gstore(list<hq_read_index_resp>(kResps) + p,
+                   hq_read_index_resp{g.cluster_id, to, index, hint, high});
     }
     __device__ __forceinline__ void state_change(uint32_t reason) {
         const uint32_t p = slot(kStates);
-        if (WRITE) list<hq_state_change>(kStates)[p] = hq_state_change{g.cluster_id, g.term, g.state, reason};
+        if (WRITE)
+            gstore(list<hq_state_change>(kStates) + p,
+                   hq_state_change{g.cluster_id, g.term, g.state, reason});
     }
     __device__ __forceinline__ void dropped(uint64_t low, uint64_t high, uint64_t from, uint32_t reason) {
         const uint32_t p = slot(kDropped);
         if (WRITE)
-            list<hq_dropped_read>(kDropped)[p] = hq_dropped_read{g.cluster_id, low, high, from, reason, 0};
+            gstore(list<hq_dropped_read>(kDropped) + p,
+                   hq_dropped_read{g.cluster_id, low, high, from, reason, 0});
     }
     __device__ __forceinline__ void defer(uint64_t e) {
         const uint32_t p = slot(kDeferred);
-        if (WRITE) list<uint64_t>(kDeferred)[p] = e;
+        if (WRITE) gstore(list<uint64_t>(kDeferred) + p, e);
     }
 
     __device__ __forceinline__ void reset(uint64_t term) {
@@ -300,7 +306,7 @@
             return true;
         }
         const int fm = member_of(from);
-        const uint32_t role = fm >= 0 ? gm[fm].role : 0xFF;
+        const uint32_t role = fm >= 0 ? gload(&gm[fm].role) : 0xFF;
         if (role == HQ_ROLE_WITNESS) {
             dropped(low, high, from, HQ_DROP_WITNESS);
             return true;
@@ -442,7 +448,7 @@
             bool dec = true;
             if (STREAM && (by_bytes || !(g.flags & kDSuspended))) dec = decode_event(br, pv, ev);
             if (by_bytes && !dec) {
-                if (!WRITE) atomicOr(a.error, (uint32_t)kErrBoffsets);
+                if (!WRITE) gor(a.error, (uint32_t)kErrBoffsets);
                 break;
             }
             if (g.flags & kDSuspended) {
@@ -453,13 +459,13 @@
             if (STREAM) {
                 ok = dec && handle(ev, e);
             } else {
-                ev = a.events[e];
+                ev = gload(a.events + e);
                 ok = handle(ev, e);
             }
             if (!ok) {
                 g.flags |= kDSuspended;
                 const uint32_t p = slot(kFallback);
-                if (WRITE) list<uint64_t>(kFallback)[p] = g.cluster_id;
+                if (WRITE) gstore(list<uint64_t>(kFallback) + p, g.cluster_id);
                 defer(e);
             } else if (STREAM && pv.run) {
                 e += take_run(pv, by_bytes ? ~0ull : e1 - e - 1);
@@ -467,15 +473,16 @@
         }
         cnt[kEvents] = (uint32_t)(e - e0);
         if (STREAM && !WRITE && !by_bytes && !(g.flags & kDSuspended) && (br.p != br.end || pv.run))
-            atomicOr(a.error, (uint32_t)kErrBoffsets);
+            gor(a.error, (uint32_t)kErrBoffsets);
         if (!WRITE && g.committed - committed0 > 0xFFFFFFFFull && a.wide)
-            atomicOr(a.wide, 1u);
+            gor(a.wide, 1u);
         if (!WRITE && a.spec_col)
-            reinterpret_cast<uint32_t *>(a.out)[i] = (uint32_t)(g.committed - committed0);
-        if (WRITE && a.layout->commit_column) {
+            gstore(reinterpret_cast<uint32_t *>(a.out) + i, (uint32_t)(g.committed - committed0));
+        if (WRITE && gload(&a.layout->commit_column)) {
         } else if (g.committed != committed0) {
             const uint32_t p = slot(kCommits);
-            if (WRITE) list<hq_commit_event>(kCommits)[p] = hq_commit_event{g.cluster_id, g.committed};
+            if (WRITE)
+                gstore(list<hq_commit_event>(kCommits) + p, hq_commit_event{g.cluster_id, g.committed});
         }
     }
 
@@ -509,24 +516,24 @@
     __device__ __forceinline__ void save_old(uint32_t h) {
         hq_dgroup o = g;
         o.pad1 = active;
-        a.groups_old[h] = o;
+        gstore(a.groups_old + h, o);
 #pragma unroll
         for (uint32_t s = 0; s < MC; ++s)
-            if (s < g.n_members) a.match_old[g.mem + s] = match[s];
-        for (uint32_t r = 0; r < g.n_reads; ++r) a.reads_old[(uint64_t)h * kDReads + r] = rd[r];
+            if (s < g.n_members) gstore(a.match_old + g.mem + s, match[s]);
+        for (uint32_t r = 0; r < g.n_reads; ++r) gstore(a.reads_old + (uint64_t)h * kDReads + r, rd[r]);
     }
 
     __device__ __forceinline__ void store(uint32_t h) {
-        a.groups[h] = g;
+        gstore(a.groups + h, g);
         hq_dmember *m = a.members + g.mem;
 #pragma unroll
         for (uint32_t s = 0; s < MC; ++s) {
             if (s < g.n_members) {
-                m[s].match = match[s];
-                m[s].active = (uint8_t)((active >> s) & 1);
-            }
-        }
-        for (uint32_t r = 0; r < g.n_reads; ++r) a.reads[(uint64_t)h * kDReads + r] = rd[r];
+                gstore(&m[s].match, match[s]);
+                gstore(&m[s].active, (uint8_t)((active >> s) & 1));
+            }
+        }
+        for (uint32_t r = 0; r < g.n_reads; ++r) gstore(a.reads + (uint64_t)h * kDReads + r, rd[r]);
     }
 };
 
@@ -606,7 +613,7 @@
             }
         }
         if (lane == 0) {
-            if (!ok) atomicOr(a.error, (uint32_t)kErrScan);
+            if (!ok) gor(a.error, (uint32_t)kErrScan);
             tile_store(a.tiles + tile, tile_word(step, chunk, true, excl + agg));
             s_excl = excl;
             s_ok = ok;
@@ -621,15 +628,15 @@
     hq_ready_to_read *dst = reinterpret_cast<hq_ready_to_read *>(a.out + a.ready_off) + lo;
     const uint32_t pos = before + x - cnt;
     if (one) {
-        const hq_ready_to_read r = a.ready_slot[i];
+        const hq_ready_to_read r = gload(a.ready_slot + i);
         if (pos < kCap) stage[pos] = r;
-        else dst[pos] = r;
+        else gstore(dst + pos, r);
     }
     __syncthreads();
     const uint32_t nq = 2 * min(agg, kCap);
     const uint4 *src = reinterpret_cast<const uint4 *>(stage);
     uint4 *out = reinterpret_cast<uint4 *>(dst);
-    for (uint32_t q = threadIdx.x; q < nq; q += 256) out[q] = src[q];
+    for (uint32_t q = threadIdx.x; q < nq; q += 256) gstore(out + q, src[q]);
 }
 
 __device__ void slot_store(const StepK &a, uint64_t tile, bool slotted, const hq_ready_compact &rec,
@@ -651,12 +658,12 @@
     char *dst = a.out + a.slot_off + tile * kSlotTileBytes;
     const uint32_t nbytes = agg * (uint32_t)sizeof(hq_ready_compact);
     for (uint32_t q = threadIdx.x; q < nbytes / 16; q += 256)
-        reinterpret_cast<uint4 *>(dst)[q] = buf[q];
+        gstore(reinterpret_cast<uint4 *>(dst) + q, buf[q]);
     if (threadIdx.x == 0) {
         if (nbytes & 8)
-            reinterpret_cast<uint2 *>(dst)[nbytes / 8 - 1] =
-                reinterpret_cast<const uint2 *>(buf)[nbytes / 8 - 1];
-        reinterpret_cast<uint32_t *>(a.out + a.cnt_off)[tile] = agg;
+            gstore(reinterpret_cast<uint2 *>(dst) + (nbytes / 8 - 1),
+                   reinterpret_cast<const uint2 *>(buf)[nbytes / 8 - 1]);
+        gstore(reinterpret_cast<uint32_t *>(a.out + a.cnt_off) + tile, agg);
     }
 }
 
@@ -667,17 +674,17 @@
     uint64_t i = a.i_begin + blk * 256 + threadIdx.x;
     constexpr bool STAGE = !WRITE && STREAM;
     bool act = true;
-    if (WRITE && (a.layout->error | a.layout->overflow)) return;
-    if (WRITE && a.layout->commit_column) {
-        if (i >= a.layout->len[kRerun]) return;
-        i = a.rerun_list[i];
+    if (WRITE && (gload(&a.layout->error) | gload(&a.layout->overflow))) return;
+    if (WRITE && gload(&a.layout->commit_column)) {
+        if (i >= gload(&a.layout->len[kRerun])) return;
+        i = gload(a.rerun_list + i);
     } else if (i >= a.i_end) {
         if (!STAGE) return;
         act = false;
     }
     uint64_t e0 = 0, e1 = 0, b0 = 0, b1 = 0;
     if (act && STREAM && a.prefix) {
-        const uint64_t x0 = a.prefix[i], x1 = a.prefix[i + 1];
+        const uint64_t x0 = gload(a.prefix + i), x1 = gload(a.prefix + i + 1);
         e0 = x0 >> 32;
         e1 = x1 >> 32;
         b0 = x0 & 0xFFFFFFFFu;
@@ -685,33 +692,33 @@
         if (!WRITE) {
             if (i + 1 == a.n && a.own_lo == 0 &&
                 ((!a.bytes_only && e1 != a.n_events) || b1 != a.n_bytes))
-                atomicOr(a.error, (uint32_t)kErrBoffsets);
+                gor(a.error, (uint32_t)kErrBoffsets);
             if (b1 < a.own_lo || b1 >= a.own_hi) act = false;
         }
     } else if (act) {
-        e0 = a.offsets[i];
-        e1 = a.offsets[i + 1];
+        e0 = gload(a.offsets + i);
+        e1 = gload(a.offsets + i + 1);
         if (STREAM) {
-            b0 = a.boffsets[i];
-            b1 = a.boffsets[i + 1];
+            b0 = gload(a.boffsets + i);
+            b1 = gload(a.boffsets + i + 1);
         }
     }
     if (!STAGE && !act) return;
     const bool member = act;
     const bool first = member && (a.prefix ? i == 0 || b0 < a.own_lo : i == a.i_begin);
-    const uint32_t h = !act ? 0u : a.handles ? a.handles[i] : (uint32_t)i;
+    const uint32_t h = !act ? 0u : a.handles ? gload(a.handles + i) : (uint32_t)i;
     if (!WRITE && act) {
         uint32_t err = 0;
         if (h >= a.n_handles) err |= kErrHandle;
         if (e1 < e0 || (!STREAM && e1 > a.n_events) || (STREAM && a.prefix && e1 > a.n_events))
             err |= kErrOffsets;
         if (STREAM && (b1 < b0 || b1 > a.n_bytes)) err |= kErrBoffsets;
-        if (!(err & kErrHandle) && atomicExch(a.stamp + h, a.step_no) == a.step_no)
+        if (!(err & kErrHandle) && gexch(a.stamp + h, a.step_no) == a.step_no)
             err |= kErrTwice;
         if (err) {
-            atomicOr(a.error, err);
-            for (int l = 0; l < kLists; ++l) a.counts[(uint64_t)l * a.n + i] = 0;
-            a.rerun[i] = 0;
+            gor(a.error, err);
+            for (int l = 0; l < kLists; ++l) gstore(a.counts + (uint64_t)l * a.n + i, 0u);
+            gstore(a.rerun + i, (uint8_t)0);
             act = false;
         }
     }
@@ -738,7 +745,7 @@
 #pragma unroll
             for (int u = 0; u < kU; ++u) {
                 const uint64_t o = (threadIdx.x + 256ull * u) * 16;
-                if (o < hi - lo) v[u] = *reinterpret_cast<const uint4 *>(lo + o);
+                if (o < hi - lo) v[u] = gload(reinterpret_cast<const uint4 *>(lo + o));
             }
 #pragma unroll
             for (int u = 0; u < kU; ++u) {
@@ -757,9 +764,10 @@
         Engine<WRITE, MC> eng(a, i, h, reads);
         if (!WRITE) eng.save_old(h);
         if (WRITE && STREAM && a.bytes_only) e0 = eng.base[kEvents];
-        if (WRITE && a.slots) eng.slotted = (a.rerun[i] & 8) != 0;
+        if (WRITE && a.slots) eng.slotted = (gload(a.rerun + i) & 8) != 0;
         __shared__ hq_ready_to_read stage[WRITE ? 256 / 64 : 1][WRITE ? kStageReady : 1];
-        const bool staged = WRITE && !a.layout->commit_column && !a.layout->ready_compact;
+        const bool staged =
+            WRITE && !gload(&a.layout->commit_column) && !gload(&a.layout->ready_compact);
         if (staged) {
             eng.stage = stage[threadIdx.x >> 6];
             eng.stage_lo = __builtin_amdgcn_readfirstlane(eng.base[kReady]);
@@ -780,7 +788,7 @@
             const uint4 *src = reinterpret_cast<const uint4 *>(eng.stage);
             uint4 *dst = reinterpret_cast<uint4 *>(eng.template list<hq_ready_to_read>(kReady) +
                                                    eng.stage_lo);
-            for (uint32_t q = rank; q < 2 * nrec; q += nact) dst[q] = src[q];
+            for (uint32_t q = rank; q < 2 * nrec; q += nact) gstore(dst + q, src[q]);
         }
         if (!WRITE) {
             const bool others = (eng.cnt[kResps] | eng.cnt[kStates] | eng.cnt[kDropped] |
@@ -788,7 +796,7 @@
             const bool rerun = others || eng.cnt[kReady] > 1;
             one_ready = !rerun && eng.cnt[kReady] == 1;
             if (a.slots && one_ready) {
-                const hq_ready_to_read r = a.ready_slot[i];
+                const hq_ready_to_read r = gload(a.ready_slot + i);
                 const int64_t delta = (int64_t)(r.index - eng.c0);
                 if (delta == (int64_t)(int32_t)delta) {
                     slotted = true;
@@ -800,8 +808,8 @@
             }
             n_ready = eng.cnt[kReady];
             eng.cnt[kRerun] = rerun;
-            for (int l = 0; l < kLists; ++l) a.counts[(uint64_t)l * a.n + i] = eng.cnt[l];
-            a.rerun[i] = (uint8_t)(2 | rerun | (one_ready ? 4 : 0) | (slotted ? 8 : 0));
+            for (int l = 0; l < kLists; ++l) gstore(a.counts + (uint64_t)l * a.n + i, eng.cnt[l]);
+            gstore(a.rerun + i, (uint8_t)(2 | rerun | (one_ready ? 4 : 0) | (slotted ? 8 : 0)));
             eng.store(h);
             uint32_t *wt = wtot[threadIdx.x >> 6];
             for (int l = 0; l < kLists; ++l)
@@ -811,7 +819,7 @@
             if ((int)(threadIdx.x & 63) == __ffsll((long long)__ballot(1)) - 1) {
                 for (int l = 0; l < kLists; ++l) {
                     const uint32_t v = wt[l];
-                    if (v) atomicAdd(a.wsum + (uint64_t)l * a.nw + (i >> 6), v);
+                    if (v) (void)gadd(a.wsum + (uint64_t)l * a.nw + (i >> 6), v);
                 }
             }
         }
@@ -825,11 +833,13 @@
 }
 
 template <bool WRITE, bool STREAM, int MC>
-__global__ __launch_bounds__(256) void k_step(const StepK a) {
+__global__ __launch_bounds__(256)
+__attribute__((amdgpu_waves_per_eu(!WRITE && !STREAM && MC == 8 ? 3 : 1)))
+void k_step(const StepK a) {
     if constexpr (!WRITE && STREAM) {
         const uint32_t b = draw_ticket(a.tickets + a.chunk);
         if (b >= gridDim.x) {
-            if (threadIdx.x == 0) atomicOr(a.error, (uint32_t)kErrTicket);
+            if (threadIdx.x == 0) gor(a.error, (uint32_t)kErrTicket);
             return;
         }
         step_groups<WRITE, STREAM, MC>(a, b, a.chunk);
@@ -842,52 +852,54 @@
 __global__ __launch_bounds__(256) void k_step_jobs(const JobMap m) {
     uint32_t b = blockIdx.x;
     if constexpr (!WRITE && STREAM) {
-        b = draw_ticket(m.tickets + m.chunk);
+        b = __builtin_amdgcn_readfirstlane(draw_ticket(m.tickets + m.chunk));
         if (b >= gridDim.x) {
-            if (threadIdx.x == 0) atomicOr(m.ks[m.job0].error, (uint32_t)kErrTicket);
+            if (threadIdx.x == 0) gor(load_job(m.ks + m.job0).error, (uint32_t)kErrTicket);
             return;
         }
     }
     const uint32_t j = job_of(m, b);
-    step_groups<WRITE, STREAM, MC>(m.ks[m.job0 + j], b - m.blk0[j], m.chunk);
+    const StepK a = load_job(m.ks + m.job0 + j);
+    step_groups<WRITE, STREAM, MC>(a, b - m.blk0[j], m.chunk);
 }
 
 __device__ __forceinline__ void lite_groups(const StepK &a, uint64_t blk, uint32_t *tickets) {
     const uint64_t i = blk * 256 + threadIdx.x;
-    if (tickets && threadIdx.x < kTickets) tickets[threadIdx.x] = 0;
-    if (i < a.ws) a.wsum[i] = 0;
+    if (tickets && threadIdx.x < kTickets) gstore(tickets + threadIdx.x, 0u);
+    if (i < a.ws) gstore(a.wsum + i, 0u);
     __shared__ __align__(16) hq_ready_to_read stage[256 / 64][kStageReady];
     static_assert(sizeof(stage) >= kSlotTileBytes, "the slot staging fits the list's");
-    if (a.slots && !a.spec_valid && !(a.layout->error | a.layout->overflow)) {
-        const bool s = i < a.n && (a.rerun[i] & 8);
+    const bool bad = (gload(&a.layout->error) | gload(&a.layout->overflow)) != 0;
+    if (a.slots && !a.spec_valid && !bad) {
+        const bool s = i < a.n && (gload(a.rerun + i) & 8);
         hq_ready_compact rec{};
         if (s) {
-            const hq_ready_to_read r = a.ready_slot[i];
-            const uint32_t h = a.handles ? a.handles[i] : (uint32_t)i;
+            const hq_ready_to_read r = gload(a.ready_slot + i);
+            const uint32_t h = a.handles ? gload(a.handles + i) : (uint32_t)i;
             rec = hq_ready_compact{r.ctx_low, r.ctx_high, (uint32_t)i,
-                                   (int32_t)(int64_t)(r.index - a.groups_old[h].committed)};
+                                   (int32_t)(int64_t)(r.index - gload(&a.groups_old[h].committed))};
         }
         slot_store(a, blk, s, rec, reinterpret_cast<uint4 *>(&stage[0][0]));
         __syncthreads();
     }
     const bool in = i < a.n;
-    if ((a.layout->error | a.layout->overflow) || !__ballot(in)) return;
-    const uint32_t col = a.layout->commit_column;
-    const uint8_t rr = in ? a.rerun[i] : 0;
+    if (bad || !__ballot(in)) return;
+    const uint32_t col = gload(&a.layout->commit_column);
+    const uint8_t rr = in ? gload(a.rerun + i) : 0;
     const int lane = threadIdx.x & 63;
     const bool replay = in && (!col || (rr & 1));
     const bool any = __ballot(replay) != 0;
     uint32_t pre_ready = 0, pre_rerun = 0;
     for (int l = 0; l < kLists; ++l) {
         if (!any && l != kReady && l != kRerun) continue;
-        const uint32_t c = in ? a.counts[(uint64_t)l * a.n + i] : 0;
+        const uint32_t c = in ? gload(a.counts + (uint64_t)l * a.n + i) : 0;
         uint32_t x = c;
 #pragma unroll
         for (int d = 1; d < 64; d <<= 1) {
             const uint32_t y = __shfl_up(x, d, 64);
             x += lane >= d ? y : 0u;
         }
-        if (replay) a.pre[(uint64_t)l * a.n + i] = x - c;
+        if (replay) gstore(a.pre + (uint64_t)l * a.n + i, x - c);
         if (l == kReady) pre_ready = x - c;
         if (l == kRerun) pre_rerun = x - c;
     }
@@ -896,53 +908,59 @@
     if (!(col32 && a.spec_valid && a.spec_ready)) {
         constexpr uint64_t l = kReady;
         const uint64_t w = i >> 6;
-        const uint32_t lo = a.scan[l * a.nw + w] - a.scan[l * a.nw];
-        const uint32_t cnt = a.scan[l * a.nw + w + 1] - a.scan[l * a.nw + w];
+        const uint32_t s_w = gload(a.scan + l * a.nw + w);
+        const uint32_t lo = s_w - gload(a.scan + l * a.nw);
+        const uint32_t cnt = gload(a.scan + l * a.nw + w + 1) - s_w;
         hq_ready_to_read *st = stage[threadIdx.x >> 6];
         const uint32_t pos = lo + pre_ready;
         const uint32_t nrec = min(cnt, kStageReady);
-        if (a.layout->ready_compact) {
+        if (gload(&a.layout->ready_compact)) {
             hq_ready_compact *stc = reinterpret_cast<hq_ready_compact *>(st);
-            hq_ready_compact *dst = reinterpret_cast<hq_ready_compact *>(a.out + a.layout->off[kReady]);
+            hq_ready_compact *dst =
+                reinterpret_cast<hq_ready_compact *>(a.out + gload(&a.layout->off[kReady]));
             if (rr & 4) {
-                const hq_ready_to_read r = a.ready_slot[i];
-                const uint32_t h = a.handles ? a.handles[i] : (uint32_t)i;
+                const hq_ready_to_read r = gload(a.ready_slot + i);
+                const uint32_t h = a.handles ? gload(a.handles + i) : (uint32_t)i;
+                const uint64_t c0 = gload(&a.groups_old[h].committed);
                 const hq_ready_compact c{r.ctx_low, r.ctx_high, (uint32_t)i,
-                                         (int32_t)(int64_t)(r.index - a.groups_old[h].committed)};
+                                         (int32_t)(int64_t)(r.index - c0)};
                 if (pos - lo < kStageReady) stc[pos - lo] = c;
-                else dst[pos] = c;
+                else gstore(dst + pos, c);
             }
             asm volatile("s_waitcnt lgkmcnt(0)" ::: "memory");
             __builtin_amdgcn_wave_barrier();
             const uint2 *src = reinterpret_cast<const uint2 *>(stc);
             uint2 *out = reinterpret_cast<uint2 *>(dst + lo);
-            for (uint32_t q = lane; q < 3 * nrec; q += 64) out[q] = src[q];
+            for (uint32_t q = lane; q < 3 * nrec; q += 64) gstore(out + q, src[q]);
         } else {
-            hq_ready_to_read *dst = reinterpret_cast<hq_ready_to_read *>(a.out + a.layout->off[kReady]);
+            hq_ready_to_read *dst =
+                reinterpret_cast<hq_ready_to_read *>(a.out + gload(&a.layout->off[kReady]));
             if (rr & 4) {
-                if (pos - lo < kStageReady) st[pos - lo] = a.ready_slot[i];
-                else dst[pos] = a.ready_slot[i];
+                const hq_ready_to_read r = gload(a.ready_slot + i);
+                if (pos - lo < kStageReady) st[pos - lo] = r;
+                else gstore(dst + pos, r);
             }
             asm volatile("s_waitcnt lgkmcnt(0)" ::: "memory");
             __builtin_amdgcn_wave_barrier();
             const uint4 *src = reinterpret_cast<const uint4 *>(st);
             uint4 *out = reinterpret_cast<uint4 *>(dst + lo);
-            for (uint32_t q = lane; q < 2 * nrec; q += 64) out[q] = src[q];
+            for (uint32_t q = lane; q < 2 * nrec; q += 64) gstore(out + q, src[q]);
         }
     }
     if (!in) return;
     if (!(col32 && a.spec_valid)) {
-        const uint32_t h = a.handles ? a.handles[i] : (uint32_t)i;
-        const uint64_t c0 = a.groups_old[h].committed, c1 = a.groups[h].committed;
-        char *cw = a.out + a.layout->off[kCommits];
+        const uint32_t h = a.handles ? gload(a.handles + i) : (uint32_t)i;
+        const uint64_t c0 = gload(&a.groups_old[h].committed), c1 = gload(&a.groups[h].committed);
+        char *cw = a.out + gload(&a.layout->off[kCommits]);
         if (col32)
-            reinterpret_cast<uint32_t *>(cw)[i] = (uint32_t)(c1 - c0);
+            gstore(reinterpret_cast<uint32_t *>(cw) + i, (uint32_t)(c1 - c0));
         else
-            reinterpret_cast<uint64_t *>(cw)[i] = c1 != c0 ? c1 : 0;
+            gstore(reinterpret_cast<uint64_t *>(cw) + i, c1 != c0 ? c1 : 0);
     }
     if (rr & 1) {
         const uint64_t l = kRerun;
-        a.rerun_list[a.scan[l * a.nw + (i >> 6)] - a.scan[l * a.nw] + pre_rerun] = (uint32_t)i;
+        const uint32_t at = gload(a.scan + l * a.nw + (i >> 6)) - gload(a.scan + l * a.nw) + pre_rerun;
+        gstore(a.rerun_list + at, (uint32_t)i);
     }
 }
 
@@ -952,23 +970,24 @@
 
 __global__ __launch_bounds__(256) void k_step_lite_jobs(const JobMap m) {
     const uint32_t j = job_of(m, blockIdx.x);
-    lite_groups(m.ks[m.job0 + j], blockIdx.x - m.blk0[j], blockIdx.x == 0 ? m.tickets : nullptr);
+    const StepK a = load_job(m.ks + m.job0 + j);
+    lite_groups(a, blockIdx.x - m.blk0[j], blockIdx.x == 0 ? m.tickets : nullptr);
 }
 
 __global__ __launch_bounds__(256) void k_step_restore(const StepK a) {
     const uint64_t i = (uint64_t)blockIdx.x * 256 + threadIdx.x;
-    if (i >= a.n || !(a.rerun[i] & 2)) return;
-    const uint32_t h = a.handles ? a.handles[i] : (uint32_t)i;
-    hq_dgroup g = a.groups_old[h];
+    if (i >= a.n || !(gload(a.rerun + i) & 2)) return;
+    const uint32_t h = a.handles ? gload(a.handles + i) : (uint32_t)i;
+    hq_dgroup g = gload(a.groups_old + h);
     const uint32_t act = g.pad1;
     g.pad1 = 0;
-    a.groups[h] = g;
+    gstore(a.groups + h, g);
     for (uint32_t s = 0; s < g.n_members; ++s) {
-        a.members[g.mem + s].match = a.match_old[g.mem + s];
-        a.members[g.mem + s].active = (uint8_t)((act >> s) & 1);
+        gstore(&a.members[g.mem + s].match, gload(a.match_old + g.mem + s));
+        gstore(&a.members[g.mem + s].active, (uint8_t)((act >> s) & 1));
     }
     for (uint32_t r = 0; r < g.n_reads; ++r)
-        a.reads[(uint64_t)h * kDReads + r] = a.reads_old[(uint64_t)h * kDReads + r];
+        gstore(a.reads + (uint64_t)h * kDReads + r, gload(a.reads_old + (uint64_t)h * kDReads + r));
 }
 
 }
```

Result: no change. 110.4 billion (-0.3%).
